# birdnet-team/birdnet-stm32

Measured on AMD Instinct MI355X. Metric: audio chunks/sec (3 s @ 24 kHz), higher is better.
Workload: dtype i8

## Files before the change

### birdnet-stm32_amd/birdnet_stm32/_hip.py

```python

from __future__ import annotations

import ctypes
import os
from ctypes import POINTER, byref, c_char_p, c_float, c_int, c_int32, c_int64, c_size_t, c_void_p

_PKG_ROOT = os.path.dirname(os.path.dirname(os.path.abspath(__file__)))
LIB_PATH = os.path.join(_PKG_ROOT, "lib", "libbirdnet_hip.so")

ABI_VERSION = 2

EXPORTS = (
    "bn_version", "bn_last_error", "bn_device_count", "bn_ctx_create", "bn_ctx_destroy", "bn_model_load",
    "bn_model_free", "bn_model_get_info", "bn_stft_mag", "bn_forward", "bn_infer_audio", "bn_debug_op_output",
    "bn_kernel_names", "bn_profile_enable", "bn_profile_collect", "bn_ingest_resample", "bn_ingest_chunks",
    "bn_pool_scores", "bn_mel_spectrogram", "bn_profile_only", "bn_chunk_peak_normalize", "bn_set_option", "bn_get_option", "bn_ctx_set_option", "bn_ctx_get_option", "bn_ctx_reset_options", "bn_preload_kernels", "bn_host_alloc_pinned", "bn_host_free_pinned", "bn_rank_orders",
    "bn_blob_check", "bn_debug_requant", "bn_stft_mag_exact", "bn_debug_input_bytes", "bn_debug_guard_stats", "bn_debug_tail_form", "bn_debug_mid_form", "bn_debug_mid_plan", "bn_debug_mid_split_giveups",
    "bn_forward_embed", "bn_infer_audio_embed", "bn_model_get_embedding_info", "bn_ingest_resample_span",
    "bn_head_forward", "bn_probe_create", "bn_probe_destroy", "bn_probe_epoch", "bn_probe_loss", "bn_probe_get", "bn_probe_set",
    "bn_probe_sweep_create", "bn_probe_sweep_destroy", "bn_probe_sweep_epoch", "bn_probe_sweep_loss", "bn_probe_sweep_snapshot", "bn_probe_sweep_get",
    "bn_probe_set_loss", "bn_probe_epoch_weighted", "bn_probe_sweep_set_loss", "bn_probe_sweep_epoch_weighted",
    "bn_probe_set_qat", "bn_probe_get_quantized", "bn_probe_scores",
    "bn_short_time_energy", "bn_activity_counts", "bn_search_inv_norms", "bn_search_topk", "bn_augment_inputs",
    "bn_kmeans_assign", "bn_kmeans_accumulate", "bn_kmeans_centroids",
    "bn_tsne_perplexity", "bn_tsne_gradient", "bn_tsne_update",
    "bn_bootstrap_rejections", "bn_bootstrap_counts", "bn_bootstrap_ap", "bn_head_i8_forward", "bn_head_i8_pass_classes",
)

EMB_F32, EMB_I8 = 0, 1
PROBE_ACTIVATIONS = {"sigmoid": 0, "softmax": 1}
PROBE_OPTIMIZERS = {"adam": 0, "adamw": 1, "sgd": 2}
PROBE_LOSSES = {"auto": 0, "focal": 1}
PROBE_QAT_WEIGHTS = {"off": 0, "per_class": 1, "per_tensor": 2}
PROBE_MAX_D, PROBE_MAX_C = 2048, 4096
PROBE_SWEEP_MAX_TRIALS = 64
PROBE_SWEEP_CURRENT, PROBE_SWEEP_SNAPSHOT = 0, 1
HEAD_I8_STEP_ROWS, HEAD_I8_MIN_WG_STEPS, HEAD_I8_MAX_WGS, HEAD_I8_LDS_BYTES = 64, 8, 1024, 160 * 1024



def head_i8_pass_classes(D: int, C: int) -> int:
    v = int(load_library().bn_head_i8_pass_classes(int(D), int(C)))
    check(min(v, 0))
    return v


class ProbeTrialStruct(ctypes.Structure):

    _fields_ = [("optimizer", ctypes.c_int32), ("lr", ctypes.c_float), ("weight_decay", ctypes.c_float), ("clipnorm", ctypes.c_float),
                ("dropout", ctypes.c_float), ("label_smoothing", ctypes.c_float)]


DTYPE_F32, DTYPE_I8 = 0, 1
SEARCH_METRICS = {"cosine": 0, "dot": 1}
SEARCH_MAX_K, SEARCH_MAX_D = 128, 2048
AUGMENT_MAX_MASKS = 4
SEARCH_STEP_ROWS, SEARCH_MIN_WG_STEPS, SEARCH_MAX_WGS = 64, 8, 1024
KMEANS_MAX_K, KMEANS_MAX_D = 4096, 2048
BOOTSTRAP_MAX_N = 32768
KMEANS_LDS_BYTES, KMEANS_MAX_TILE, KMEANS_STEP_ROWS, KMEANS_MIN_WG_STEPS, KMEANS_MAX_WGS, KMEANS_SEGMENT_ROWS = 160 * 1024, 128, 64, 8, 1024, 256
TSNE_TILE_I, TSNE_TILE_J, TSNE_SPLIT_J, TSNE_ROW_LANES, TSNE_MAX_K, TSNE_MAX_N = 256, 1024, 4096, 16, 128, 1 << 21


def kmeans_tile_centroids(D: int, K: int) -> int:
    pitch_bytes = (-(-int(D) // 64) * 64 + 4) * 4
    nt = 1
    while nt < KMEANS_MAX_TILE // 16 and 16 * nt < K:
        nt *= 2
    while nt > 1 and 16 * nt * pitch_bytes > KMEANS_LDS_BYTES:
        nt //= 2
    return 16 * nt


OPTION_NAMES = ("f32_strip", "f32_strip_th", "f32_front_staged", "f32_front2", "f32_pwdw", "f32_tile_slice", "f32_pw_ws", "i8_pwdw", "i8_pw_lds", "i8_pw_forms", "i8_add_tab", "front_tpw", "wave_dwpw", "i8_strip", "i8_strip_mfdw", "i8_strip_th", "i8_dw_pool", "i8_tail_fclds", "i8_tail", "i8_tail_mfdw", "i8_mid",
                "i8_mel_generic", "stft_rowmajor", "stft_exact", "stft_flagcap", "stft_guard", "stft_audit", "stft_minint", "ingest_blk", "ingest_generic")
SCHEDULING_OPTION_NAMES = ("i8_mid_split",)


class BnModelInfo(ctypes.Structure):
    _fields_ = [
        ("dtype", c_int32), ("input_kind", c_int32), ("input_elems", c_int32), ("fft_bins", c_int32),
        ("spec_width", c_int32), ("num_classes", c_int32), ("n_ops", c_int32), ("max_batch", c_int32),
        ("workspace_bytes", c_int64), ("const_bytes", c_int64),
    ]


class HipError(RuntimeError):
    """A libbirdnet_hip call returned a negative status."""


_lib = None


def load_library(path: str | None = None):
    global _lib
    if _lib is not None:
        return _lib
    path = path or os.environ.get("BIRDNET_HIP_LIB", LIB_PATH)
    if not os.path.isfile(path):
        raise RuntimeError(
            f"{path} not found: the HIP extension has not been built. Run `python -c 'import __graft_entry__ as g; "
            "g.build()'` (or `make -C birdnet-stm32_amd/csrc`). There is no CPU fallback for this path."
        )
    import torch

    lib = ctypes.CDLL(path)
    for name in EXPORTS:
        if not hasattr(lib, name):
            raise RuntimeError(f"{path} does not export {name}")
    lib.bn_version.restype = c_int
    lib.bn_last_error.restype = c_char_p
    lib.bn_device_count.restype = c_int
    lib.bn_ctx_create.argtypes = [c_int, c_int, POINTER(c_void_p)]
    lib.bn_ctx_destroy.argtypes = [c_void_p]
    lib.bn_ctx_destroy.restype = None
    lib.bn_model_load.argtypes = [c_void_p, c_char_p, c_size_t, POINTER(c_void_p)]
    lib.bn_model_free.argtypes = [c_void_p]
    lib.bn_model_free.restype = None
    lib.bn_model_get_info.argtypes = [c_void_p, POINTER(BnModelInfo)]
    lib.bn_stft_mag.argtypes = [c_void_p, c_void_p, c_int, c_int, c_int, c_int, c_int, c_int, c_void_p, c_void_p, c_void_p]
    lib.bn_stft_mag_exact.argtypes = lib.bn_stft_mag.argtypes
    lib.bn_debug_input_bytes.argtypes = [c_void_p, c_int, c_void_p, c_void_p]
    lib.bn_debug_guard_stats.argtypes = [c_void_p, c_int, POINTER(c_int64)]
    lib.bn_debug_tail_form.argtypes = [c_void_p, POINTER(c_int), POINTER(c_int)]
    lib.bn_debug_mid_form.argtypes = [c_void_p, POINTER(c_int), POINTER(c_int)]
    lib.bn_debug_mid_plan.argtypes = [c_void_p, POINTER(c_int), c_int]
    lib.bn_debug_mid_split_giveups.argtypes = [c_void_p, POINTER(c_int64)]
    lib.bn_forward.argtypes = [c_void_p, c_void_p, c_void_p, c_int, c_void_p, c_void_p, c_void_p]
    lib.bn_infer_audio.argtypes = [c_void_p, c_void_p, c_int, c_int, c_int, c_void_p, c_void_p, c_void_p]
    lib.bn_forward_embed.argtypes = [c_void_p, c_void_p, c_void_p, c_int, c_void_p, c_void_p, c_void_p, c_int, c_void_p]
    lib.bn_infer_audio_embed.argtypes = [c_void_p, c_void_p, c_int, c_int, c_int, c_void_p, c_void_p, c_void_p, c_int, c_void_p]
    lib.bn_model_get_embedding_info.argtypes = [c_void_p, POINTER(c_int), POINTER(c_int), POINTER(c_float), POINTER(c_int)]
    lib.bn_debug_op_output.argtypes = [c_void_p, c_int, c_int, c_void_p, c_size_t, POINTER(c_size_t), c_void_p]
    lib.bn_kernel_names.restype = c_char_p
    lib.bn_profile_enable.argtypes = [c_void_p, c_int]
    lib.bn_profile_only.argtypes = [c_void_p, c_int]
    lib.bn_chunk_peak_normalize.argtypes = [c_void_p, c_void_p, c_int, c_int, c_float, c_void_p, c_void_p]
    lib.bn_profile_collect.argtypes = [c_void_p, POINTER(ctypes.c_double), POINTER(c_int64), c_int]
    lib.bn_ingest_resample.argtypes = [c_void_p, c_void_p, c_int, c_int, c_void_p, c_void_p, c_int, c_int64, c_int64,
                                       c_void_p, c_int, c_int, c_int, c_int, c_void_p, c_void_p, c_void_p]
    lib.bn_ingest_resample_span.argtypes = [c_void_p, c_void_p, c_int, c_int, c_int64, c_int64, c_int64, c_int64, c_int64, c_void_p,
                                            c_int, c_int, c_int, c_int, c_void_p, c_void_p, c_void_p]
    lib.bn_ingest_chunks.argtypes = [c_void_p, c_void_p, c_void_p, c_void_p, c_void_p, c_void_p, c_int, c_int, c_void_p,
                                     c_void_p]
    lib.bn_pool_scores.argtypes = [c_void_p, c_void_p, c_void_p, c_int, c_int, c_int, c_float, c_void_p, c_void_p]
    lib.bn_mel_spectrogram.argtypes = [c_void_p, c_void_p, c_int, c_int, c_int, c_int, c_int, c_void_p, c_void_p, c_int, c_int, c_int,
                                       ctypes.c_double, c_void_p, c_int, c_void_p, c_void_p, c_void_p]
    lib.bn_blob_check.argtypes = [c_char_p, c_size_t]
    lib.bn_debug_requant.argtypes = [c_void_p, c_void_p, c_void_p, c_void_p, c_int, c_int, c_int, c_void_p, c_void_p]
    lib.bn_set_option.argtypes = [c_char_p, c_int]
    lib.bn_get_option.argtypes = [c_char_p, POINTER(c_int)]
    lib.bn_ctx_set_option.argtypes = [c_void_p, c_char_p, c_int]
    lib.bn_ctx_get_option.argtypes = [c_void_p, c_char_p, POINTER(c_int)]
    lib.bn_ctx_reset_options.argtypes = [c_void_p]
    lib.bn_preload_kernels.argtypes = [c_void_p]
    lib.bn_rank_orders.argtypes = [c_void_p, c_void_p, c_int, c_int, c_void_p, c_void_p, c_void_p]
    lib.bn_short_time_energy.argtypes = [c_void_p, c_void_p, c_void_p, c_void_p, c_void_p, c_void_p, c_int, c_int, c_int, c_void_p, c_void_p]
    lib.bn_activity_counts.argtypes = [c_void_p, c_void_p, c_int, c_int64, c_void_p, c_int, c_float, c_void_p, c_void_p, c_void_p]
    lib.bn_search_inv_norms.argtypes = [c_void_p, c_void_p, c_int, c_int64, c_int, c_int, c_void_p, c_void_p]
    lib.bn_search_topk.argtypes = [c_void_p, c_void_p, c_int, c_int64, c_int, c_int, c_void_p, c_void_p, c_int64, c_void_p, c_int, c_void_p, c_void_p,
                                   c_int, c_void_p, c_void_p, c_void_p]
    lib.bn_kmeans_assign.argtypes = [c_void_p, c_void_p, c_int, c_int64, c_int, c_int, c_void_p, c_void_p, c_void_p, c_int, c_void_p, c_void_p, c_void_p,
                                     c_void_p, c_void_p]
    lib.bn_kmeans_accumulate.argtypes = [c_void_p, c_void_p, c_int, c_int64, c_int, c_int, c_void_p, c_void_p, c_int, c_int, c_void_p, c_void_p, c_void_p]
    lib.bn_kmeans_centroids.argtypes = [c_void_p, c_void_p, c_void_p, c_int, c_int, c_void_p, c_void_p, c_void_p]
    lib.bn_tsne_perplexity.argtypes = [c_void_p, c_void_p, c_int64, c_int, ctypes.c_double, c_void_p, c_void_p, c_void_p]
    lib.bn_tsne_gradient.argtypes = [c_void_p, c_void_p, c_int64, c_void_p, c_void_p, c_void_p, c_float, c_void_p, c_void_p, c_void_p, c_void_p]
    lib.bn_tsne_update.argtypes = [c_void_p, c_void_p, c_void_p, c_void_p, c_void_p, c_int64, c_float, c_float, c_void_p]
    u64 = ctypes.c_uint64
    lib.bn_bootstrap_rejections.argtypes = [c_void_p, u64, u64, u64, u64, ctypes.c_uint32, c_int64, c_int64, c_void_p, c_int64, POINTER(c_int64), c_void_p]
    lib.bn_bootstrap_counts.argtypes = [c_void_p, u64, u64, u64, u64, c_int, c_int, c_void_p, c_void_p, c_void_p]
    lib.bn_bootstrap_ap.argtypes = [c_void_p, u64, u64, u64, u64, c_int, c_int, c_void_p, c_void_p, c_void_p, c_void_p, c_int, c_int, c_void_p, c_void_p, c_void_p]
    lib.bn_augment_inputs.argtypes = [c_void_p, c_void_p, c_int64, c_int, c_int, c_void_p, c_void_p, c_void_p, c_void_p, c_int, c_void_p, c_int, c_int64,
                                      c_void_p, c_void_p]
    lib.bn_host_alloc_pinned.argtypes = [c_void_p, ctypes.c_size_t]
    lib.bn_host_alloc_pinned.restype = c_void_p
    lib.bn_host_free_pinned.argtypes = [c_void_p]
    lib.bn_head_forward.argtypes = [c_void_p, c_void_p, c_int64, c_int, c_void_p, c_void_p, c_int, c_int, c_void_p, c_void_p]
    lib.bn_head_i8_forward.argtypes = [c_void_p, c_void_p, c_int64, c_int, c_void_p, c_void_p, c_void_p, c_void_p, c_int, c_int, c_void_p, c_int, c_float,
                                       c_void_p, c_void_p, c_void_p]
    lib.bn_head_i8_pass_classes.argtypes = [c_int, c_int]
    lib.bn_probe_create.argtypes = [c_void_p, c_int, c_int, c_int, c_int, c_float, c_float, c_float, c_float, ctypes.c_uint32, c_int64,
                                    c_void_p, c_void_p, POINTER(c_void_p), c_void_p]
    lib.bn_probe_destroy.argtypes = [c_void_p]
    lib.bn_probe_destroy.restype = None
    lib.bn_probe_epoch.argtypes = [c_void_p, c_void_p, c_void_p, c_void_p, c_int64, c_int, c_void_p, c_void_p]
    lib.bn_probe_loss.argtypes = [c_void_p, c_void_p, c_void_p, c_int64, c_void_p, c_void_p]
    lib.bn_probe_get.argtypes = [c_void_p, c_void_p, c_void_p, c_void_p]
    lib.bn_probe_set.argtypes = [c_void_p, c_void_p, c_void_p, c_void_p]
    lib.bn_probe_sweep_create.argtypes = [c_void_p, c_int, c_int, c_int, c_int, POINTER(ProbeTrialStruct), ctypes.c_uint32, c_int64, c_void_p, c_void_p,
                                          POINTER(c_void_p), c_void_p]
    lib.bn_probe_sweep_destroy.argtypes = [c_void_p]
    lib.bn_probe_sweep_destroy.restype = None
    lib.bn_probe_sweep_epoch.argtypes = [c_void_p, c_void_p, c_void_p, c_void_p, c_int64, c_int, c_void_p, c_void_p, c_void_p, c_void_p]
    lib.bn_probe_sweep_loss.argtypes = [c_void_p, c_void_p, c_void_p, c_int64, c_void_p, c_void_p, c_void_p]
    lib.bn_probe_sweep_snapshot.argtypes = [c_void_p, c_void_p, c_void_p]
    lib.bn_probe_sweep_get.argtypes = [c_void_p, c_int, c_int, c_void_p, c_void_p, c_void_p]
    lib.bn_probe_set_loss.argtypes = [c_void_p, c_int, c_float]
    lib.bn_probe_epoch_weighted.argtypes = [c_void_p, c_void_p, c_void_p, c_void_p, c_void_p, c_int64, c_int, c_void_p, c_void_p]
    lib.bn_probe_sweep_set_loss.argtypes = [c_void_p, c_int, c_float]
    lib.bn_probe_set_qat.argtypes = [c_void_p, c_int, c_int, c_float, c_int]
    lib.bn_probe_get_quantized.argtypes = [c_void_p, c_void_p, c_void_p]
    lib.bn_probe_scores.argtypes = [c_void_p, c_void_p, c_int64, c_void_p, c_void_p, c_void_p]
    lib.bn_probe_sweep_epoch_weighted.argtypes = [c_void_p, c_void_p, c_void_p, c_void_p, c_void_p, c_int64, c_int, c_void_p, c_void_p, c_void_p, c_void_p]
    if lib.bn_version() != ABI_VERSION:
        raise RuntimeError(f"libbirdnet_hip ABI {lib.bn_version()} != binding ABI {ABI_VERSION}")
    _lib = lib
    return lib

# ... 121 lines not shown
```

### birdnet-stm32_amd/birdnet_stm32/models/runners.py

```python

from __future__ import annotations

import ctypes

import numpy as np

from birdnet_stm32 import _hip
from birdnet_stm32.models import _pack as pk


class HipRunner:

    def __init__(self, plan: pk.Plan, device: int = 0, max_batch: int = 1024, ctx: "_hip.Context | None" = None):
        import torch

        if not torch.cuda.is_available():
            raise RuntimeError("no ROCm device visible: HipRunner has no CPU fallback")
        self._torch = torch
        self.plan = plan
        self.device = torch.device("cuda", device)
        self.ctx = ctx if ctx is not None else _hip.Context(device, max_batch)
        self.model = _hip.Model(self.ctx, plan.to_blob())
        self.lib = self.ctx.lib
        info = self.model.info
# ... 145 lines not shown
    def infer_audio_device(self, audio, hop: int | None = None, return_logits: bool = False, out=None, return_embeddings: bool = False,
                           emb_dtype: str = "float32", emb_out=None):
        torch = self._torch
        self._check_dev(audio, "audio")
        kw = dict(return_embeddings=True, emb_dtype=emb_dtype, emb_out=emb_out) if return_embeddings else {}
        if self.input_kind in (pk.INPUT_MEL, pk.INPUT_WAVEFORM):
            res = self.predict_device(self.model_inputs_device(audio), return_logits=return_logits, **kw)
            if out is not None:
                out.copy_(res[0] if isinstance(res, tuple) else res)
            return res
        B, T = audio.shape
        hop = int(hop) if hop is not None else T // self.spec_width
        scores = out if out is not None else torch.empty((B, self.num_classes), dtype=torch.float32, device=self.device)
        logits = torch.empty_like(scores) if return_logits else None
        emb, code = (None, 0)
        if return_embeddings:
            emb, code = self._emb_buffer(B, emb_dtype, emb_out)
        with torch.cuda.device(self.device):
            for b0 in range(0, B, self.max_batch):
                nb = min(self.max_batch, B - b0)
                if emb is not None:
                    _hip.check(self.lib.bn_infer_audio_embed(self.model.handle, audio[b0:].data_ptr(), nb, T, hop, scores[b0:].data_ptr(),
                                                             logits[b0:].data_ptr() if logits is not None else None, emb[b0:].data_ptr(), code,
                                                             self._stream()))
                    continue
                _hip.check(
                    self.lib.bn_infer_audio(
                        self.model.handle, audio[b0:].data_ptr(), nb, T, hop, scores[b0:].data_ptr(),
                        logits[b0:].data_ptr() if logits is not None else None, self._stream(),
                    )
                )
        if emb is not None:
            return (scores, logits, emb) if return_logits else (scores, emb)
        return (scores, logits) if return_logits else scores

    def stft_device(self, audio, n_fft: int = 512, hop: int | None = None, spec_width: int | None = None, normalize: bool = True,
                    exact: bool = False):
        return stft_device(self.ctx, audio, n_fft, hop, spec_width or self.spec_width, normalize, exact=exact)

    def op_output(self, op_index: int, B: int) -> np.ndarray:
        torch = self._torch
        op = self.plan.ops[op_index]
        per = ctypes.c_size_t()
        _hip.check(self.lib.bn_debug_op_output(self.model.handle, op_index, B, None, 0, ctypes.byref(per), None))
        buf = torch.empty((B, per.value), dtype=torch.uint8, device=self.device)
        _hip.check(self.lib.bn_debug_op_output(self.model.handle, op_index, B, buf.data_ptr(), buf.numel(), ctypes.byref(per), self._stream()))
        torch.cuda.synchronize(self.device)
        raw = buf.cpu().numpy().reshape(-1)
        n = int(np.prod(op.out_shape))
        dt = np.dtype(op.out_dtype)
        return raw[: B * n * dt.itemsize].copy().view(dt).reshape(B, *op.out_shape)

    def input_bytes(self, B: int) -> np.ndarray:
        torch = self._torch
        out = torch.empty((B, self.fft_bins, self.spec_width), dtype=torch.int8, device=self.device)
        _hip.check(self.lib.bn_debug_input_bytes(self.model.handle, B, out.data_ptr(), self._stream()))
        torch.cuda.synchronize(self.device)
        return out.cpu().numpy()

    def guard_stats(self, B: int) -> dict:
        out = (ctypes.c_int64 * 8)()
        _hip.check(self.lib.bn_debug_guard_stats(self.model.handle, B, out))
        return {"listed": int(out[0]), "listed_max": int(out[1]), "dirty_blocks": int(out[2]), "whole_minmax": int(out[3]), "whole_fix": int(out[4]),
                "audited": int(out[5]), "audit_violations": int(out[6]), "interval_min": int(out[7])}

    def tail_form(self) -> tuple[int, int]:
        form, lds = ctypes.c_int(0), ctypes.c_int(0)
        _hip.check(self.lib.bn_debug_tail_form(self.model.handle, ctypes.byref(form), ctypes.byref(lds)))
        return form.value, lds.value

    def mid_form(self) -> tuple[int, int]:
        form, lds = ctypes.c_int(0), ctypes.c_int(0)
        _hip.check(self.lib.bn_debug_mid_form(self.model.handle, ctypes.byref(form), ctypes.byref(lds)))
        return form.value, lds.value

    def mid_plan(self) -> dict | None:
        out = (ctypes.c_int * 64)()
        _hip.check(self.lib.bn_debug_mid_plan(self.model.handle, out, 64))
        if not out[0]:
            return None
        parts = [(out[5 + 6 * i + 2 * k], out[6 + 6 * i + 2 * k]) for i in range(out[4]) for k in range(3) if out[6 + 6 * i + 2 * k]]
        return {"lds_bytes": out[1], "map_bytes": out[2], "bar_off": out[3], "blocks": out[4], "parts": parts}

    def mid_split_giveups(self) -> int:
        n = ctypes.c_int64(0)
        _hip.check(self.lib.bn_debug_mid_split_giveups(self.ctx.handle, ctypes.byref(n)))
        return int(n.value)

    def profile(self, enable: bool) -> None:
        _hip.check(self.lib.bn_profile_enable(self.model.handle, int(bool(enable))))

    def profile_only(self, op_index: int) -> None:
        _hip.check(self.lib.bn_profile_only(self.model.handle, int(op_index)))

    def profile_collect(self) -> list[dict]:
        n = len(self.plan.ops) + 3
        ms = (ctypes.c_double * n)()
        cnt = (ctypes.c_int64 * n)()
        _hip.check(self.lib.bn_profile_collect(self.model.handle, ms, cnt, n))
        rows = []
        for i in range(n):
            if i < len(self.plan.ops):
                op = self.plan.ops[i]
                rows.append({"op": i, "kind": pk.KIND_NAMES[op.kind], "name": op.name, "ms": ms[i], "launches": int(cnt[i]), "p": list(op.p)})
            else:
                kind, name = (("stft512", "stft"), ("stft_minmax_exact", "exact min/max"), ("stft512_f64_list", "float64 pass + redo"))[i - len(self.plan.ops)]
                rows.append({"op": i, "kind": kind, "name": name, "ms": ms[i], "launches": int(cnt[i]), "p": []})
        return rows

    def close(self):
        import sys

        pl = sys.modules.get("birdnet_stm32.audio.pipeline")
        if pl is not None:
            while pl._PREPARE:
                pl._PREPARE.pop().join()
        self.model.close()
        self.ctx.close()


def stft_device(ctx: _hip.Context, audio, n_fft: int = 512, hop: int | None = None, spec_width: int = 256, normalize: bool = True,
                return_minmax: bool = False, exact: bool = False):
    import torch

    if not (audio.is_cuda and audio.dtype == torch.float32 and audio.is_contiguous() and audio.dim() == 2):
        raise ValueError("audio must be a contiguous float32 CUDA tensor [B, T]")
    B, T = audio.shape
    hop = int(hop) if hop is not None else T // spec_width
    spec = torch.empty((B, n_fft // 2 + 1, spec_width), dtype=torch.float32, device=audio.device)
    minmax = torch.empty((B, 2), dtype=torch.float32, device=audio.device)
    with torch.cuda.device(audio.device):
        stream = ctypes.c_void_p(torch.cuda.current_stream(audio.device).cuda_stream)
        fn = ctx.lib.bn_stft_mag_exact if exact else ctx.lib.bn_stft_mag
        _hip.check(fn(ctx.handle, audio.data_ptr(), B, T, n_fft, hop, spec_width, int(normalize), spec.data_ptr(), minmax.data_ptr(), stream))
    return (spec, minmax) if return_minmax else spec


def lower_model_file(model_path: str, keep_all: bool = False, frontend_norm: bool | None = None, fuse: bool = True) -> pk.Plan:
    if model_path.lower().endswith(".tflite"):
        from birdnet_stm32.models._lower_i8 import lower_i8
        from birdnet_stm32.models._tflite_reader import load_tflite

        return lower_i8(load_tflite(model_path), keep_all=keep_all, fuse=fuse)
    from birdnet_stm32.models._keras_loader import load_keras_archive
    from birdnet_stm32.models._lower_f32 import lower_f32

    return lower_f32(load_keras_archive(model_path, frontend_norm=frontend_norm), keep_all=keep_all, fuse=fuse)


def load_model_runner(model_path: str, device: int = 0, max_batch: int = 1024, keep_all: bool = False,
                      frontend_norm: bool | None = None, fuse: bool = True, prepare_pipeline: bool = False) -> HipRunner:
    ctx = None
    if prepare_pipeline:
        import torch

        if not torch.cuda.is_available():
            raise RuntimeError("no ROCm device visible: HipRunner has no CPU fallback")
        from birdnet_stm32.audio.pipeline import prepare_for_evaluate

        ctx = _hip.Context(device, max_batch)
        prepare_for_evaluate(ctx, torch)
    plan = lower_model_file(model_path, keep_all=keep_all, frontend_norm=frontend_norm, fuse=fuse)
    return HipRunner(plan, device=device, max_batch=max_batch, ctx=ctx)
```

### birdnet-stm32_amd/csrc/bn_api.hip

```cpp
#include <hip/hip_runtime.h>

#include <algorithm>
#include <cctype>
#include <cmath>
#include <cstdarg>
#include <cstdio>
#include <cstdlib>
#include <cstring>
#include <string>
#include <vector>

#include "bn_model.h"

namespace {

thread_local std::string g_err;

constexpr int kFft = 512;

struct OptName {
    const char* name;
    int bn::Options::*field;
};
const OptName kOptions[] = {
    {"f32_strip", &bn::Options::f32_strip},       {"f32_strip_th", &bn::Options::f32_strip_th},
    {"f32_front_staged", &bn::Options::f32_front_staged}, {"f32_front2", &bn::Options::f32_front2}, {"f32_pwdw", &bn::Options::f32_pwdw}, {"f32_tile_slice", &bn::Options::f32_tile_slice}, {"f32_pw_ws", &bn::Options::f32_pw_ws}, {"i8_pwdw", &bn::Options::i8_pwdw}, {"i8_pw_lds", &bn::Options::i8_pw_lds}, {"i8_pw_forms", &bn::Options::i8_pw_forms}, {"i8_add_tab", &bn::Options::i8_add_tab}, {"front_tpw", &bn::Options::front_tpw},
    {"wave_dwpw", &bn::Options::wave_dwpw},       {"i8_strip", &bn::Options::i8_strip},
    {"i8_strip_th", &bn::Options::i8_strip_th}, {"i8_dw_pool", &bn::Options::i8_dw_pool}, {"i8_tail_fclds", &bn::Options::i8_tail_fclds},   {"i8_tail", &bn::Options::i8_tail}, {"i8_tail_mfdw", &bn::Options::i8_tail_mfdw}, {"i8_mid", &bn::Options::i8_mid}, {"i8_mid_split", &bn::Options::i8_mid_split},
    {"i8_mel_generic", &bn::Options::i8_mel_generic}, {"stft_rowmajor", &bn::Options::stft_rowmajor},
    {"i8_strip_mfdw", &bn::Options::i8_strip_mfdw}, {"stft_exact", &bn::Options::stft_exact}, {"stft_flagcap", &bn::Options::stft_flagcap}, {"stft_guard", &bn::Options::stft_guard}, {"stft_audit", &bn::Options::stft_audit}, {"stft_minint", &bn::Options::stft_minint},
    {"ingest_blk", &bn::Options::ingest_blk},
    {"ingest_generic", &bn::Options::ingest_generic},
};

bn::Options options_from_env() {
    bn::Options o;
    for (const OptName& e : kOptions) {
        std::string var = "BN_";
        for (const char* c = e.name; *c; ++c) var += (char)toupper((unsigned char)*c);
        if (const char* v = getenv(var.c_str())) o.*(e.field) = atoi(v);
    }
    return o;
}

}

namespace bn {
thread_local Options g_opt;

int fail(int code, const char* fmt, ...) {
    char buf[512];
    va_list ap;
    va_start(ap, fmt);
    vsnprintf(buf, sizeof buf, fmt, ap);
    va_end(ap);
    g_err = buf;
    return code;
}
}
using bn::fail;
using bn::kMaxGridBatch;
using bn::ProfScope;

bn::Options g_opt_default = options_from_env();
std::mutex g_opt_mu;

namespace bn {

int check_device(bn_ctx* ctx) {
    if (!ctx) return fail(BN_ERR_ARG, "null context");
    HIP_TRY(hipSetDevice(ctx->device));
    {
        std::lock_guard<std::mutex> lock(g_opt_mu);
        bn::g_opt = g_opt_default;
        for (const auto& ov : ctx->opt_override) bn::g_opt.*(ov.first) = ov.second;
    }
    return BN_OK;
}

int grow_device_buffer(void** p, size_t* have, size_t need, size_t alloc, hipStream_t s, int code, const char* what) {
    if (need <= *have) return BN_OK;
    HIP_TRY(hipStreamSynchronize(s));
    if (*p) (void)hipFree(*p);
    *p = nullptr;
    *have = 0;
    if (hipMalloc(p, alloc) != hipSuccess) {
        (void)hipGetLastError();
        return fail(code, "hipMalloc of %zu bytes for the %s workspace failed", alloc, what);
    }
    *have = alloc;
    return BN_OK;
}

}
using bn::check_device;
using bn::grow_device_buffer;

namespace {

int row_matrix_check(int dtype, int64_t n, int D, int max_D, int zero_point) {
    if (dtype != BN_DTYPE_F32 && dtype != BN_DTYPE_I8) return fail(BN_ERR_ARG, "unknown dtype %d", dtype);
    if (D < 1 || D > max_D) return fail(BN_ERR_ARG, "embedding width D=%d outside 1..%d", D, max_D);
    if (n < 0 || n > 0x7fffffffLL) return fail(BN_ERR_ARG, "bad row count %lld", (long long)n);
    if (dtype == BN_DTYPE_I8 && (zero_point < -128 || zero_point > 127)) return fail(BN_ERR_ARG, "zero point %d outside -128..127", zero_point);
    return BN_OK;
}

}

extern "C" {

// ... 93 lines not shown
    if (c->d_tsne_work) (void)hipFree(c->d_tsne_work);
    if (c->d_boot_work) (void)hipFree(c->d_boot_work);
    delete c;
}

static int parse_blob(const void* blob, size_t nbytes, BlobHeader& h, std::vector<SlotRec>& slots, std::vector<TensorRec>& tensors,
                      std::vector<OpRec>& ops) {
    if (!blob || nbytes < sizeof(BlobHeader)) return fail(BN_ERR_FORMAT, "blob too small (%zu bytes)", nbytes);
    const char* base = (const char*)blob;
    memcpy(&h, base, sizeof h);
    if (memcmp(h.magic, BN_BLOB_MAGIC, 8) != 0) return fail(BN_ERR_FORMAT, "bad blob magic");
    if (h.version != BN_BLOB_VERSION)
        return fail(BN_ERR_FORMAT, "blob version %u, library expects %u", h.version, BN_BLOB_VERSION);
    auto in_range = [&](uint64_t off, uint64_t len) { return off <= nbytes && len <= nbytes - off; };
    if (!in_range(h.slots_off, (uint64_t)h.n_slots * sizeof(SlotRec)) ||
        !in_range(h.tensors_off, (uint64_t)h.n_tensors * sizeof(TensorRec)) ||
        !in_range(h.ops_off, (uint64_t)h.n_ops * sizeof(OpRec)))
        return fail(BN_ERR_FORMAT, "blob tables exceed the blob size");
    slots.resize(h.n_slots);
    tensors.resize(h.n_tensors);
    ops.resize(h.n_ops);
    if (h.n_slots) memcpy(slots.data(), base + h.slots_off, h.n_slots * sizeof(SlotRec));
    if (h.n_tensors) memcpy(tensors.data(), base + h.tensors_off, h.n_tensors * sizeof(TensorRec));
    if (h.n_ops) memcpy(ops.data(), base + h.ops_off, h.n_ops * sizeof(OpRec));
    for (const TensorRec& t : tensors)
        if (!in_range(t.offset, t.nbytes) || (t.offset & 255)) return fail(BN_ERR_FORMAT, "tensor payload out of range or misaligned");
    for (const SlotRec& sl : slots)
        if (sl.bytes_per_chunk > (1ull << 32)) return fail(BN_ERR_FORMAT, "slot of %llu bytes per chunk", (unsigned long long)sl.bytes_per_chunk);
    for (const OpRec& o : ops) {
        for (int k = 0; k < BN_OP_NT; ++k)
            if (o.t[k] >= (int)h.n_tensors) return fail(BN_ERR_FORMAT, "operator references tensor %d of %u", o.t[k], h.n_tensors);
        const int ids[3] = {o.in0, o.in1, o.out};
        for (int id : ids)
            if (id >= (int)h.n_slots || (id < 0 && id != BN_SLOT_INPUT && id != BN_SLOT_SCORES && id != BN_SLOT_LOGITS && id != BN_SLOT_AUDIO && id != BN_SLOT_NONE))
                return fail(BN_ERR_FORMAT, "operator references slot %d of %u", id, h.n_slots);
    }
    std::string why;
    if (!bn::check_plan(h, slots, tensors, ops, why)) return fail(BN_ERR_FORMAT, "%s", why.c_str());
    return BN_OK;
}

int bn_blob_check(const void* blob, size_t nbytes) {
    BlobHeader h;
    std::vector<SlotRec> slots;
    std::vector<TensorRec> tensors;
    std::vector<OpRec> ops;
    return parse_blob(blob, nbytes, h, slots, tensors, ops);
}

int bn_model_load(bn_ctx* ctx, const void* blob, size_t nbytes, bn_model** out) {
    if (!out) return fail(BN_ERR_ARG, "out is null");
    *out = nullptr;
    if (int rc = check_device(ctx)) return rc;
    bn_model* m = new bn_model();
    m->ctx = ctx;
    if (int rc = parse_blob(blob, nbytes, m->hdr, m->slots, m->tensors, m->ops)) {
        delete m;
        return rc;
    }
    if (int rc = bn::prepare_plan(m, blob)) {
        delete m;
        return rc;
    }
    const BlobHeader& h = m->hdr;
    const char* base = (const char*)blob;
    size_t lo = nbytes, hi = 0;
    for (const TensorRec& t : m->tensors)
        if (t.nbytes) {
            lo = t.offset < lo ? (size_t)t.offset : lo;
            hi = t.offset + t.nbytes > hi ? (size_t)(t.offset + t.nbytes) : hi;
        }
    auto cleanup_fail = [&](int code) {
        bn_model_free(m);
        return code;
    };
    if (hi > lo) {
        m->consts_base = lo;
        m->consts_bytes = hi - lo;
        if (hipMalloc(&m->d_consts, m->consts_bytes) != hipSuccess)
            return cleanup_fail(fail(BN_ERR_NOMEM, "hipMalloc of %zu constant bytes failed", m->consts_bytes));
        if (hipMemcpy(m->d_consts, base + lo, m->consts_bytes, hipMemcpyHostToDevice) != hipSuccess)
            return cleanup_fail(fail(BN_ERR_DEVICE, "copying constants to the device failed"));
    }
    const size_t mb = (size_t)ctx->max_batch;
    m->d_slots.assign(h.n_slots, nullptr);
    for (uint32_t i = 0; i < h.n_slots; ++i) {
        const size_t bytes = mb * m->slots[i].bytes_per_chunk;
        if (bytes == 0) continue;
        if (hipMalloc(&m->d_slots[i], bytes) != hipSuccess)
            return cleanup_fail(fail(BN_ERR_NOMEM, "hipMalloc of %zu workspace bytes (slot %u) failed", bytes, i));
        m->workspace_bytes += bytes;
    }
    if (h.input_kind == BN_INPUT_SPECTROGRAM) {
        const size_t bytes = mb * h.input_elems * sizeof(float);
        if (hipMalloc(&m->d_spec, bytes) != hipSuccess)
            return cleanup_fail(fail(BN_ERR_NOMEM, "hipMalloc of %zu spectrogram workspace bytes failed", bytes));
        m->workspace_bytes += bytes;
    }
    if (m->guard_form_ok && h.dtype == BN_DTYPE_I8) {
        const size_t W = h.spec_width, n_tiles = (W + 15) / 16, t64 = (W + 63) / 64;
        const int cap = 1 << 20;
        size_t off = 0;
        auto take = [&](size_t bytes) {
            const size_t o = off;
            off += (bytes + 255) & ~(size_t)255;
            return o;
        };
        const size_t o_eps = take(mb * W * 4), o_rec = take(mb * n_tiles * bn::kGuardRec * 4), o_list = take(mb * 4), o_cnt = take(mb * 4),
                     o_dirty = take(mb * 4), o_work = take(mb * t64 * 4), o_nw = take(4 * (mb / kMaxGridBatch + 1)), o_hard = take(2 * mb * 4),
                     o_nh = take(8 * (mb / kMaxGridBatch + 1)), o_audit = take(8);
        if (hipMalloc(&m->d_guard, off) != hipSuccess) return cleanup_fail(fail(BN_ERR_NOMEM, "hipMalloc of %zu exactness-pass bytes failed", off));
        m->workspace_bytes += off;
        char* g = m->d_guard;
        m->guard = bn::StftGuard{(float*)(g + o_eps), (int*)(g + o_rec), (float*)(g + o_list), (int*)(g + o_cnt), cap, (int*)(g + o_dirty),
                                 (int*)(g + o_work), (int*)(g + o_nw), (int*)(g + o_hard), (int*)(g + o_nh), (int)mb};
        m->d_audit = (int*)(g + o_audit);
    }
    if (hipMalloc(&m->d_minmax, mb * 2 * sizeof(float)) != hipSuccess ||
        hipMalloc(&m->d_smax, mb * sizeof(float)) != hipSuccess)
        return cleanup_fail(fail(BN_ERR_NOMEM, "hipMalloc of reduction scratch failed"));
    m->workspace_bytes += mb * 3 * sizeof(float);
    if (m->pool8_C) {
        if (hipMalloc(&m->d_pool8, mb * m->pool8_C * sizeof(int32_t)) != hipSuccess)
            return cleanup_fail(fail(BN_ERR_NOMEM, "hipMalloc of pooling scratch failed"));
        if (hipMemset(m->d_pool8, 0, mb * m->pool8_C * sizeof(int32_t)) != hipSuccess) return cleanup_fail(fail(BN_ERR_DEVICE, "clearing the pooling scratch failed"));
        m->workspace_bytes += mb * m->pool8_C * sizeof(int32_t);
    }
    if (m->gap_part_elems) {
        if (hipMalloc(&m->d_gap_part, mb * m->gap_part_elems * sizeof(float)) != hipSuccess)
            return cleanup_fail(fail(BN_ERR_NOMEM, "hipMalloc of pooling scratch failed"));
        m->workspace_bytes += mb * m->gap_part_elems * sizeof(float);
    }
    *out = m;
    return BN_OK;
}

void bn_model_free(bn_model* m) {
    if (!m) return;
    if (m->ctx) (void)hipSetDevice(m->ctx->device);
    (void)hipFree(m->d_consts);
    for (char* p : m->d_slots) (void)hipFree(p);
    (void)hipFree(m->d_spec);
    (void)hipFree(m->d_minmax);
    (void)hipFree(m->d_guard);
    (void)hipFree(m->d_smax);
    (void)hipFree(m->d_gap_part);
    (void)hipFree(m->d_pool8);
    for (auto& r : m->ev_used) {
        (void)hipEventDestroy(r.start);
        (void)hipEventDestroy(r.stop);
    }
    for (hipEvent_t e : m->ev_free) (void)hipEventDestroy(e);
    delete m;
}

int bn_model_get_info(const bn_model* m, bn_model_info* out) {
    if (!m || !out) return fail(BN_ERR_ARG, "null argument");
    out->dtype = (int32_t)m->hdr.dtype;
    out->input_kind = (int32_t)m->hdr.input_kind;
    out->input_elems = (int32_t)m->hdr.input_elems;
    out->fft_bins = (int32_t)m->hdr.fft_bins;
    out->spec_width = (int32_t)m->hdr.spec_width;
    out->num_classes = (int32_t)m->hdr.num_classes;
    out->n_ops = (int32_t)m->hdr.n_ops;
    out->max_batch = m->ctx->max_batch;
    out->workspace_bytes = (int64_t)m->workspace_bytes;
    out->const_bytes = (int64_t)m->consts_bytes;
    return BN_OK;
}

static int stft_mag_impl(bn_ctx* ctx, const float* d_audio, int B, int T, int n_fft, int hop, int W, int normalize, float* d_spec,
                         float* d_minmax, void* stream, bool tile_major, bool exact = false);

int bn_stft_mag(bn_ctx* ctx, const float* d_audio, int B, int T, int n_fft, int hop, int W, int normalize,
                float* d_spec, float* d_minmax, void* stream) {
    return stft_mag_impl(ctx, d_audio, B, T, n_fft, hop, W, normalize, d_spec, d_minmax, stream, false);
}

int bn_stft_mag_exact(bn_ctx* ctx, const float* d_audio, int B, int T, int n_fft, int hop, int W, int normalize,
                      float* d_spec, float* d_minmax, void* stream) {
    return stft_mag_impl(ctx, d_audio, B, T, n_fft, hop, W, normalize, d_spec, d_minmax, stream, false, true);
}

static int stft_mag_impl(bn_ctx* ctx, const float* d_audio, int B, int T, int n_fft, int hop, int W, int normalize, float* d_spec,
                         float* d_minmax, void* stream, bool tile_major, bool exact) {
    if (int rc = check_device(ctx)) return rc;
    if (!d_audio || !d_spec || !d_minmax) return fail(BN_ERR_ARG, "null device pointer");
    if (n_fft != kFft) return fail(BN_ERR_UNSUPPORTED, "n_fft=%d: only 512 is implemented", n_fft);
    if (B < 0 || T <= 0 || W <= 0 || hop <= 0) return fail(BN_ERR_ARG, "bad shape B=%d T=%d hop=%d W=%d", B, T, hop, W);
    if (1 + T / hop < W)
        return fail(BN_ERR_ARG, "T=%d hop=%d gives %d frames, fewer than spec_width=%d", T, hop, 1 + T / hop, W);
    if (B == 0) return BN_OK;
    hipStream_t s = (hipStream_t)stream;
    const size_t per_chunk = (size_t)(kFft / 2 + 1) * W;
    for (int b0 = 0; b0 < B; b0 += kMaxGridBatch) {
        const int nb = B - b0 < kMaxGridBatch ? B - b0 : kMaxGridBatch;
        bn::launch_minmax_init(d_minmax + 2 * (size_t)b0, nb, s);
        if (exact)
            bn::launch_stft512_f64(ctx->tables, d_audio + (size_t)b0 * T, nb, T, hop, W, d_spec + b0 * per_chunk, d_minmax + 2 * (size_t)b0, s,
                                   tile_major);
        else
            bn::launch_stft512(ctx->tables, d_audio + (size_t)b0 * T, nb, T, hop, W, d_spec + b0 * per_chunk,
                               d_minmax + 2 * (size_t)b0, s, tile_major);
        if (normalize)
            bn::launch_spec_normalize(d_spec + b0 * per_chunk, d_minmax + 2 * (size_t)b0, nb, (int)per_chunk, s);
    }
    HIP_TRY(hipGetLastError());
    return BN_OK;
}

int bn_mel_spectrogram(bn_ctx* ctx, const float* d_audio, int B, int T, int n_fft, int hop, int W, const float* d_mel_w,
                       const int32_t* d_mel_bands, int n_mels, int mode, int mag_scale, double pcen_b, const float* d_dct,
                       int n_mfcc, float* d_work, float* d_out, void* stream) {
    if (int rc = check_device(ctx)) return rc;
    if (!d_audio || !d_mel_w || !d_mel_bands || !d_work || !d_out) return fail(BN_ERR_ARG, "null device pointer");
    if (n_fft != kFft) return fail(BN_ERR_UNSUPPORTED, "n_fft=%d: only 512 is implemented", n_fft);
    if (B < 0 || T <= 0 || W <= 0 || hop <= 0 || n_mels <= 0) return fail(BN_ERR_ARG, "bad shape B=%d T=%d hop=%d W=%d mels=%d", B, T, hop, W, n_mels);
    if (1 + T / hop < W)
        return fail(BN_ERR_ARG, "T=%d hop=%d gives %d frames, fewer than spec_width=%d", T, hop, 1 + T / hop, W);
    if (mode < BN_SPEC_MEL || mode > BN_SPEC_MFCC) return fail(BN_ERR_ARG, "unknown spectrogram mode %d", mode);
    if (mag_scale < BN_MAG_NONE || mag_scale > BN_MAG_DB) return fail(BN_ERR_ARG, "unknown mag_scale %d", mag_scale);
    if (mode != BN_SPEC_MEL) mag_scale = BN_MAG_NONE;
    if (mode == BN_SPEC_MFCC && (!d_dct || n_mfcc <= 0 || n_mfcc > n_mels)) return fail(BN_ERR_ARG, "mfcc needs 0 < n_mfcc <= n_mels and a DCT matrix");
// ... 116 lines not shown
                                 d_emb ? (char*)d_emb + b0 * D * esize : nullptr, emb_dtype, (hipStream_t)stream, d_audio + (size_t)b0 * T, T, hop};
            if (int rc = bn::run_plan(m, ra)) return rc;
        }
        return BN_OK;
    }
    if (int rc = check_device(m->ctx)) return rc;
    if (!d_audio || !d_scores) return fail(BN_ERR_ARG, "null device pointer");
    if (B == 0) return BN_OK;
    const bool tiled = m->spec_tiled_ok && !bn::g_opt.stft_rowmajor;
    hipStream_t s = (hipStream_t)stream;
    const size_t in_stride = m->hdr.input_elems, C = m->hdr.num_classes;
    const bool i8 = m->hdr.dtype == BN_DTYPE_I8;
    const int exact_opt = i8 ? bn::g_opt.stft_exact : 0;
    const bool guarded = exact_opt == 2 && tiled && m->d_guard && !bn::g_opt.i8_mel_generic && W % 16 == 0 && W <= 1024;
    int rc = BN_OK;
    if (guarded) {
        if (T <= 0 || hop <= 0 || 1 + T / hop < W) rc = fail(BN_ERR_ARG, "T=%d hop=%d gives %d frames, fewer than spec_width=%d", T, hop, hop > 0 ? 1 + T / hop : 0, W);
        if (m->d_audit) HIP_TRY(hipMemsetAsync(m->d_audit, 0, 2 * sizeof(int), s));
        for (int b0 = 0; rc == BN_OK && b0 < B; b0 += kMaxGridBatch) {
            const int nb = B - b0 < kMaxGridBatch ? B - b0 : kMaxGridBatch;
            bn::StftGuard g = bn::guard_slice(m, (size_t)b0, bn::SpecStage{tiled, true, d_audio + (size_t)b0 * T, T, hop});
            {
                ProfScope prof(m, (int)m->ops.size(), s);
                bn::launch_stft512(m->ctx->tables, d_audio + (size_t)b0 * T, nb, T, hop, W, m->d_spec + b0 * in_stride, m->d_minmax + 2 * (size_t)b0, s,
                                   true, &g);
            }
            ProfScope prof(m, (int)m->ops.size() + 1, s);
            bn::launch_stft_minmax_exact(m->ctx->tables, d_audio + (size_t)b0 * T, nb, T, hop, W, m->d_spec + b0 * in_stride, true, g,
                                         m->d_minmax + 2 * (size_t)b0, s);
        }
    } else {
        ProfScope prof(m, (int)m->ops.size(), s);
        rc = stft_mag_impl(m->ctx, d_audio, B, T, kFft, hop, W, 0, m->d_spec, m->d_minmax, stream, tiled, exact_opt != 0);
    }
    if (rc == BN_OK) {
        for (int b0 = 0; b0 < B; b0 += kMaxGridBatch) {
            const int nb = B - b0 < kMaxGridBatch ? B - b0 : kMaxGridBatch;
            bn::RunArgs ra{m->d_spec + b0 * in_stride, m->d_minmax + 2 * (size_t)b0, nb, d_scores + b0 * C, d_logits ? d_logits + b0 * C : nullptr,
                           d_emb ? (char*)d_emb + b0 * D * esize : nullptr, emb_dtype, s};
            ra.slot_b0 = (size_t)b0;
            ra.spec = bn::SpecStage{tiled, guarded, d_audio + (size_t)b0 * T, T, hop};
            rc = bn::run_plan(m, ra);
            if (rc != BN_OK) break;
        }
    }
    m->last_tiled = tiled;
    m->last_B = rc == BN_OK ? B : 0;
    return rc;
}

extern "C" {

int bn_debug_tail_form(const bn_model* m, int* form, int* lds_bytes) {
    if (!m || !form || !lds_bytes) return fail(BN_ERR_ARG, "null argument");
    *form = 0;
    *lds_bytes = 0;
    for (size_t oi = 0; oi < m->ops.size(); ++oi) {
        if (m->ops[oi].kind != BN_OP_I8_TAIL || !m->prep[oi]->ok) continue;
        const bn::OpPrep& pr = *m->prep[oi];
        *form = pr.alt_ok ? 2 : 1;
        *lds_bytes = pr.alt_ok ? pr.chain.lds_bytes : pr.tail.lds_bytes;
    }
    return BN_OK;
}

int bn_debug_mid_form(const bn_model* m, int* form, int* lds_bytes) {
    if (!m || !form || !lds_bytes) return fail(BN_ERR_ARG, "null argument");
    *form = 0;
    *lds_bytes = 0;
    for (size_t oi = 0; oi < m->ops.size(); ++oi)
        if (m->ops[oi].kind == BN_OP_I8_MID && m->prep[oi]->ok) {
            *form = 1;
            *lds_bytes = m->prep[oi]->chain.lds_bytes;
        }
    return BN_OK;
}

int bn_debug_mid_plan(const bn_model* m, int* out, int n) {
    if (!m || !out || n < 1) return fail(BN_ERR_ARG, "null argument");
    out[0] = 0;
    for (size_t oi = 0; oi < m->ops.size(); ++oi)
        if (m->ops[oi].kind == BN_OP_I8_MID && m->prep[oi]->ok && m->prep[oi]->alt_ok) {
            if (!bn::tail2_plan_dump(m->prep[oi]->resident, out, n)) return fail(BN_ERR_ARG, "n=%d is too small for the plan", n);
            break;
        }
    return BN_OK;
}

int bn_debug_mid_split_giveups(bn_ctx* ctx, int64_t* count) {
    if (!ctx || !count) return fail(BN_ERR_ARG, "null argument");
    if (int rc = check_device(ctx)) return rc;
    const long n = bn::tail2_giveups();
    if (n < 0) return fail(BN_ERR_DEVICE, "could not read the chunk barriers' give-up counter");
    *count = n;
    return BN_OK;
}

int bn_debug_guard_stats(bn_model* m, int B, int64_t* out) {
    if (!m || !out) return fail(BN_ERR_ARG, "null argument");
    if (int rc = check_device(m->ctx)) return rc;
    if (!m->d_guard) return fail(BN_ERR_UNSUPPORTED, "the plan has no exactness pass");
    if (B <= 0 || B > m->last_B || B > kMaxGridBatch) return fail(BN_ERR_ARG, "B=%d: the last bn_infer_audio call left %d spectrograms", B, m->last_B);
    HIP_TRY(hipDeviceSynchronize());
    std::vector<int> cnt((size_t)B);
    int nw = 0, nh[2] = {0, 0};
    HIP_TRY(hipMemcpy(cnt.data(), m->guard.count, (size_t)B * sizeof(int), hipMemcpyDeviceToHost));
    HIP_TRY(hipMemcpy(&nw, m->guard.n_work, sizeof(int), hipMemcpyDeviceToHost));
    HIP_TRY(hipMemcpy(nh, m->guard.n_hard, 2 * sizeof(int), hipMemcpyDeviceToHost));
    int64_t total = 0, mx = 0;
    for (int c : cnt) {
        c %= m->guard.cap + 1;
        total += c;
        if (c > mx) mx = c;
    }
    out[0] = total;
    out[1] = mx;
    out[2] = nw;
    out[3] = nh[0];
    out[4] = nh[1];
    int au[2] = {0, 0};
    if (m->d_audit) HIP_TRY(hipMemcpy(au, m->d_audit, sizeof au, hipMemcpyDeviceToHost));
    out[5] = au[0];
    out[6] = au[1];
    std::vector<float> lo((size_t)B);
    HIP_TRY(hipMemcpy(lo.data(), m->guard.mn_lo, (size_t)B * sizeof(float), hipMemcpyDeviceToHost));
    int64_t wide = 0;
    for (float v : lo) wide += v >= 0.0f;
    out[7] = wide;
    return BN_OK;
}

int bn_debug_input_bytes(bn_model* m, int B, int8_t* d_out, void* stream) {
    if (!m || !d_out) return fail(BN_ERR_ARG, "null argument");
    if (int rc = check_device(m->ctx)) return rc;
    namespace k = bn::op::i8_dwpw;
    const OpRec* first = nullptr;
    for (const OpRec& o : m->ops)
        if (o.in0 == BN_SLOT_INPUT && o.kind == BN_OP_I8_DWPW && o.p[k::q_at_load] && o.p[k::transposed]) first = &o;
    if (!first || !m->d_spec) return fail(BN_ERR_UNSUPPORTED, "the plan's first operator is not the mel mixer with QUANTIZE fused into its load");
    if (B <= 0 || B > m->last_B || B > kMaxGridBatch) return fail(BN_ERR_ARG, "B=%d: the last bn_infer_audio call left %d spectrograms", B, m->last_B);
    bn::launch_spec_bytes(m->d_spec, m->d_minmax, B, (int)m->hdr.spec_width, m->last_tiled, first->f[k::qscale], first->p[k::qzp], d_out, (hipStream_t)stream);
    HIP_TRY(hipGetLastError());
    return BN_OK;
}

int bn_ingest_resample(bn_ctx* ctx, const void* d_pcm, int sample_format, int channels, const int64_t* d_in_off,
                       const int64_t* d_out_off, int n_windows, int64_t max_in_len, int64_t max_out_len, const float* d_taps,
                       int up, int down, int taps_per_phase, int n_pre_remove, float* d_mono, float* d_peak, void* stream) {
    if (int rc = check_device(ctx)) return rc;
    if (!d_pcm || !d_in_off || !d_out_off || !d_mono || !d_peak) return fail(BN_ERR_ARG, "null device pointer");
    if (sample_format < BN_PCM_S16 || sample_format > BN_PCM_F32) return fail(BN_ERR_ARG, "unknown sample format %d", sample_format);
    if (channels < 1 || channels > 8)
        return fail(BN_ERR_UNSUPPORTED, "%d channels: the channel mean is implemented for 1..8 channels", channels);
    if (n_windows < 0 || max_in_len < 0 || max_out_len < 0 || up < 1 || down < 1 || taps_per_phase < 0 || n_pre_remove < 0)
        return fail(BN_ERR_ARG, "bad ingest geometry");
    if (taps_per_phase > 0 && !d_taps) return fail(BN_ERR_ARG, "null filter");
    if (taps_per_phase == 0 && up != down) return fail(BN_ERR_ARG, "up=%d down=%d needs a filter", up, down);
    if (n_windows == 0 || max_out_len == 0) return BN_OK;
    if (n_windows > 65535) return fail(BN_ERR_ARG, "at most 65535 windows per call");
    if ((double)(max_out_len + n_pre_remove + 4096) * down >= 4294967296.0 || (double)max_in_len * up >= 4294967296.0)
        return fail(BN_ERR_UNSUPPORTED, "window too long for the 32-bit polyphase index (%lld samples, up=%d, down=%d)",
                    (long long)max_in_len, up, down);
    const size_t lds = bn::ingest_resample_lds_bytes(up, down, taps_per_phase, bn::ingest_resample_block(up, down, taps_per_phase));
    const bool fast_kernel = (up == 1 && (down == 2 || down == 4)) || (up > 1 && up <= 256 && (taps_per_phase == 21 || taps_per_phase == 29 || taps_per_phase == 39));
    if (lds > (fast_kernel ? 64 : 156) * 1024)
        return fail(BN_ERR_UNSUPPORTED, "resampling ratio %d/%d needs %zu bytes of LDS per workgroup (limit %d)", up, down, lds, (fast_kernel ? 64 : 156) * 1024);
// ... 605 lines not shown
```

### birdnet-stm32_amd/csrc/bn_chain_plan.cpp

```cpp
#include "bn_chain_plan.h"

#include <algorithm>
#include <vector>

namespace bn {
namespace {

constexpr int kLdsCap = 160 * 1024;
#ifdef BN_TAIL_STAMPS
constexpr int kStampBytes = 16;
#else
constexpr int kStampBytes = 0;
#endif

struct Span {
    int b, e;
};
bool overlap(Span p, Span q) { return p.b < q.e && q.b < p.e; }
int first_fit(std::vector<Span>& used, int bytes, int cap) {
    bytes = (bytes + 15) & ~15;
    int pos = 0;
    for (;;) {
        bool moved = false;
        for (const Span& s : used)
// ... 89 lines not shown
    return true;
}

long tail_const_words(const Tail8Args& a) {
    long need = 0;
    auto upto = [&](long off, long words) { need = off + words > need ? off + words : need; };
    for (int i = 0; i < a.n_layers; ++i) {
        const Tail8Layer& L = a.L[i];
        upto(L.g_w, (long)L.Cin * L.Cout / 4);
        upto(L.g_dwc, (long)L.Cin * 7);
        upto(L.g_pwc, (long)L.Cout * 4);
        if (L.has_add) upto(L.g_lut, 512);
    }
    upto(a.g_fcw, (long)a.NC * a.C / 4);
    upto(a.g_fcb, a.NC);
    upto(a.g_fcm, a.NC);
    upto(a.g_fcs, a.NC);
    if (a.g_hlut >= 0) upto(a.g_hlut, 64);
    return need;
}

namespace {

Span dw_span(const Tail2Layer& L, bool first) { return {L.dw_off, L.dw_off + tail2_dw_bytes(L, first)}; }
int tail2_map_bytes(const Tail2Layer& L, bool first, int G) {
    return std::max(first ? 0 : G * L.H * L.W * (L.Cin + 16), G * L.OH * L.OW * (L.Cout + 16));
}
void tail2_place_counters(Tail2Args& a) {
    a.bar_off = (a.lds_bytes + 15) & ~15;
    if (a.bar_off + 16 > kLdsCap) a.bar_off = -1;
    else a.lds_bytes = a.bar_off + 16;
}

}

bool tail2_plan(const int32_t* desc, int n_words, int n_layers, Tail2Args& a, bool mid) {
    constexpr int LW = kTail2LayerWords, CAP = kLdsCap - kStampBytes;
    const int HW = mid ? 0 : kTailHeadWords, G = mid ? kMidG : kTailG;
    if (n_layers < 1 || n_layers > 8 || n_words != LW * n_layers + HW) return false;
    a.n_layers = n_layers;
    int lds_need = 0;
    Span prev_pw{0, 0}, map_last{0, 0};
    auto grow = [&](int end) { lds_need = end > lds_need ? end : lds_need; };
    for (int attempt = 0; attempt < 2; ++attempt) {
        lds_need = 0;
        prev_pw = {0, 0};
        for (int i = 0; i < n_layers; ++i) {
            const int32_t* d = desc + LW * i;
            Tail2Layer& L = a.L[i];
            read_layer(d, L);
            L.res_m = d[20]; L.res_c_lo = d[21]; L.res_c_hi = d[22]; L.res_k = d[23]; L.g_cst = d[24];
            const bool first = i == 0;
            if (!(mid ? shape_ok(a.L, i, kMidShapes) : shape_ok(a.L, i, kTailShapes))) return false;
            if (L.g_cst < 0 || (L.g_cst & 3)) return false;
            if (first && L.zp_in != -128) return false;
            if (!int8_range(L.dw_lo, L.dw_hi) || L.pw_lo > L.pw_hi) return false;
            if (!L.has_add && !int8_range(L.pw_lo, L.pw_hi)) return false;
            if (L.has_add && (!int8_range(L.add_lo, L.add_hi) || L.add_e < 1 || L.add_e > 22 || L.add_m < 0 || L.res_m < 0 || L.res_k < 3 || L.res_k > 19))
                return false;
            if (tail2_dw_bytes(L, first) / 16 > kTail2MaxDw16) return false;
            const Span map{0, tail2_map_bytes(L, first, G)};
            L.x_off = first ? -1 : 0;
            L.y_off = 0;
            std::vector<Span> used{map};
            if (prev_pw.e > prev_pw.b) used.push_back(prev_pw);
            L.zp_off = first ? 0 : first_fit(used, L.Cin + 16, CAP);
            if (L.zp_off < 0) return false;
            L.dw_off = first && attempt ? (CAP - tail2_dw_bytes(L, first)) & ~15 : first_fit(used, tail2_dw_bytes(L, first), CAP);
            if (L.dw_off < 0) return false;
            used = {map, dw_span(L, first)};
            if (!first) used.push_back({L.zp_off, L.zp_off + L.Cin + 16});
            L.pw_off = first_fit(used, tail2_pw_bytes(L), CAP);
            if (L.pw_off < 0) return false;
            prev_pw = {L.pw_off, L.pw_off + tail2_pw_bytes(L)};
            grow(map.e); grow(dw_span(L, first).e); grow(prev_pw.e);
        }
        const Tail2Layer& last = a.L[n_layers - 1];
        map_last = {0, G * last.OH * last.OW * (last.Cout + 16)};
        if (!overlap(dw_span(a.L[0], true), map_last) && !overlap(dw_span(a.L[0], true), prev_pw)) break;
        if (attempt) return false;
    }
    const Tail2Layer& last = a.L[n_layers - 1];
    a.resident = 0;
    a.bar_off = -1;
    a.fcw_off = -1;
    if (mid) {
        a.P = last.OH * last.OW;
        a.C = last.Cout;
        a.lds_bytes = lds_need;
        tail2_place_counters(a);
        return a.C % 16 == 0;
    }
    read_head(desc + LW * n_layers, a);
    if (a.g_fcw < 0 || a.g_fcb < 0 || a.g_hlut < -1 || (a.g_fcw & 3) || (a.g_fcb & 3)) return false;
    if (!int8_range(a.fc_lo, a.fc_hi)) return false;
    if (a.P != last.OH * last.OW || a.C != last.Cout || a.C % 64 || a.C > 256 || a.NC < 1 || (a.NC + 15) / 16 > kTail2Waves) return false;
    std::vector<Span> used{map_last, dw_span(a.L[0], true)};
    a.mean_off = first_fit(used, kTailG * last.Cout, CAP);
    if (a.mean_off < 0) return false;
    grow(a.mean_off + kTailG * last.Cout);
    a.lds_bytes = lds_need;
    tail2_place_counters(a);
    return true;
}

bool tail2_plan_resident(Tail2Args& a) {
    if (a.n_layers < 1 || a.n_layers > 8) return false;
    int map_bytes = 0;
    for (int i = 0; i < a.n_layers; ++i) map_bytes = std::max(map_bytes, tail2_map_bytes(a.L[i], i == 0, kMidG));
    std::vector<Span> used{{0, map_bytes}};
    for (int i = 0; i < a.n_layers; ++i) {
        Tail2Layer& L = a.L[i];
        if (tail2_dw_bytes(L, i == 0) / 16 > kTail2MaxDw16 || tail2_pw_bytes(L) / 16 > kTail2MaxDw16) return false;
        if ((L.dw_off = first_fit(used, tail2_dw_bytes(L, i == 0), kLdsCap)) < 0) return false;
        if ((L.pw_off = first_fit(used, tail2_pw_bytes(L), kLdsCap)) < 0) return false;
        L.zp_off = 0;
        if (i > 0 && (L.zp_off = first_fit(used, L.Cin + 16, kLdsCap)) < 0) return false;
    }
    if ((a.bar_off = first_fit(used, 16, kLdsCap)) < 0) return false;
    for (size_t i = 0; i < used.size(); ++i)
        for (size_t j = i + 1; j < used.size(); ++j)
            if (overlap(used[i], used[j])) return false;
    const Tail2Layer& last = a.L[a.n_layers - 1];
    if (last.OH != 16 || last.OW != 32 || last.Cout != 64 || a.P != 16 * 32 || a.C != 64) return false;
    int end = 0;
    for (const Span& u : used) end = std::max(end, u.e);
    a.lds_bytes = end;
    a.resident = 1;
    return end <= kLdsCap;
}

bool tail2_plan_dump(const Tail2Args& a, int* out, int n) {
    if (n < 5 + 6 * a.n_layers) return false;
    int map_bytes = 0;
    for (int i = 0; i < a.n_layers; ++i) {
        const Tail2Layer& L = a.L[i];
        map_bytes = std::max(map_bytes, tail2_map_bytes(L, i == 0, kMidG));
        int* o = out + 5 + 6 * i;
        o[0] = L.dw_off; o[1] = tail2_dw_bytes(L, i == 0); o[2] = L.pw_off; o[3] = tail2_pw_bytes(L); o[4] = L.zp_off; o[5] = i == 0 ? 0 : L.Cin + 16;
    }
    out[0] = a.resident; out[1] = a.lds_bytes; out[2] = map_bytes; out[3] = a.bar_off; out[4] = a.n_layers;
    return true;
}

long tail2_const_words(const Tail2Args& a, bool mid) {
    long need = 0;
    auto upto = [&](long off, long words) { need = off + words > need ? off + words : need; };
    for (int i = 0; i < a.n_layers; ++i) upto(a.L[i].g_cst, (tail2_dw_bytes(a.L[i], i == 0) + tail2_pw_bytes(a.L[i])) / 4);
    if (mid) return need;
    const long nct = (a.NC + 15) / 16;
    upto(a.g_fcw, nct * (a.C / 64) * 256);
    upto(a.g_fcb, nct * 48);
    if (a.g_hlut >= 0) upto(a.g_hlut, 64);
    return need;
}

}
```

### birdnet-stm32_amd/csrc/bn_chain_plan.h

```cpp
#pragma once
#include <stdint.h>

#if defined(__HIPCC__)
#define BN_HOST_DEVICE __host__ __device__
#else
#define BN_HOST_DEVICE
#endif

namespace bn {

constexpr int kTailG = 4;
constexpr int kTailWaves = 16;
constexpr int kTailThreads = 64 * kTailWaves;
constexpr int kTailLayerWords = 24;
constexpr int kTailHeadWords = 16;
struct Tail8Layer {
    int H, W, Cin, Cout, S, OH, OW, pt, pl, has_add;
    int zp_in, dw_lo, dw_hi, pw_lo, pw_hi;
    int add_m, add_c1, add_e, add_lo, add_hi;
    int g_w, g_dwc, g_pwc, g_lut;
    int x_off, y_off, w_off, dwc_off, pwc_off, lut_off, zp_off;
};
struct Tail8Args {
    const int8_t* x;
    float* scores;
    float* logits;
    const int32_t* cst;
    int B, n_layers, NC, P, C;
    int mean_zp_in, mean_mult, mean_shift, mean_zp_out, mean_off;
    int fc_zp_out, fc_lo, fc_hi, g_fcw, g_fcb, g_fcm, g_fcs, g_hlut, head_zp_fc, head_zp_out;
    float s_fc, s_head;
    int lds_bytes;
    int fcw_off;
    Tail8Layer L[8];};
bool tail_plan(const int32_t* desc, int n_words, int n_layers, Tail8Args& a);
long tail_const_words(const Tail8Args& a);

constexpr int kTail2Waves = 8;
constexpr int kTail2Threads = 64 * kTail2Waves;
constexpr int kTail2LayerWords = 32;
struct Tail2Layer {
    int H, W, Cin, Cout, S, OH, OW, pt, pl, has_add;
    int zp_in, dw_lo, dw_hi, pw_lo, pw_hi;
    int add_m, add_c1, add_e, add_lo, add_hi;
    int res_m, res_c_lo, res_c_hi, res_k;
    int g_cst;
    int x_off, y_off, dw_off, pw_off, zp_off;
};
constexpr int kMidG = 2;
struct Tail2Args {
    const int8_t* x;
    int8_t* y;
    float* scores;
    float* logits;
    const int32_t* cst;
    int B, n_layers, NC, P, C;
    int mean_zp_in, mean_mult, mean_shift, mean_zp_out, mean_off;
    int fc_zp_out, fc_lo, fc_hi, g_fcw, g_fcb, g_fcm, g_fcs, g_hlut, head_zp_fc, head_zp_out;
    float s_fc, s_head;
    int lds_bytes;
    int fcw_off;
    int bar_off;
    int resident;
    Tail2Layer L[8];};
constexpr int kTail2MaxDw16 = 7 * kTail2Threads;
BN_HOST_DEVICE inline int tail2_dw_bytes(const Tail2Layer& L, bool first) { return (L.Cin / 16) * (3 * 1024 + (first ? 8 : 5) * 64); }
BN_HOST_DEVICE inline int tail2_pw_bytes(const Tail2Layer& L) { return (L.Cin + 63) / 64 * 64 * L.Cout + (L.Cout / 16) * 5 * 64; }
bool tail2_plan(const int32_t* desc, int n_words, int n_layers, Tail2Args& a, bool mid = false);
bool tail2_plan_resident(Tail2Args& a);
bool tail2_plan_dump(const Tail2Args& a, int* out, int n);
long tail2_const_words(const Tail2Args& a, bool mid = false);

}
```

### birdnet-stm32_amd/csrc/bn_i8_tail2.hip

```cpp
#include "bn_tail_common.h"

namespace bn {
namespace {

#ifdef BN_TAIL_STAMPS
__device__ long long* g_tail2_stamps = nullptr;
__device__ long long* g_mid2_stamps = nullptr;
#define BN_T2STAMP(i) do { if ((i) != 7) st[i] = (long long)__builtin_amdgcn_s_memrealtime(); } while (0)
#else
#define BN_T2STAMP(i) do {} while (0)
#endif

__device__ __forceinline__ long upair(uint32_t lo, uint32_t hi) { return (long)(((unsigned long)hi << 32) | lo); }

template <int MAXP>
__device__ __forceinline__ void part_request(const int32_t* src, unsigned char* dst, int n16, int tid) {
    const int wave = __builtin_amdgcn_readfirstlane(tid >> 6);
#pragma unroll
    for (int i = 0; i < MAXP; ++i) {
        const int idx = i * kTail2Threads + tid;
        if (idx < n16)
            __builtin_amdgcn_global_load_lds((const __attribute__((address_space(1))) void*)(src + 4 * (size_t)idx),
                                             (__attribute__((address_space(3))) void*)(dst + (i * kTail2Threads + wave * 64) * 16), 16, 0, 0);
    }
}
__device__ unsigned g_tail2_giveups = 0;
#ifdef BN_TAIL_STAMPS
constexpr bool kStamped = true;
#else
constexpr bool kStamped = false;
#endif
template <int WPC>
__device__ __forceinline__ void chunk_barrier(unsigned char* lds, int bar_off, int slot, unsigned& seq) {
    unsigned* ctr = reinterpret_cast<unsigned*>(lds + bar_off) + slot;
    seq += 1;
    const unsigned target = (unsigned)WPC * seq;
    asm volatile("s_waitcnt lgkmcnt(0)" ::: "memory");
    __builtin_amdgcn_fence(__ATOMIC_RELEASE, "workgroup", "local");
    if ((threadIdx.x & 63) == 0) __hip_atomic_fetch_add(ctr, 1u, __ATOMIC_RELAXED, __HIP_MEMORY_SCOPE_WORKGROUP);
    bool done = false;
#pragma unroll 1
    for (int spins = 0; spins < (1 << 20); ++spins) {
        const unsigned v = (unsigned)__builtin_amdgcn_readfirstlane((int)__hip_atomic_load(ctr, __ATOMIC_RELAXED, __HIP_MEMORY_SCOPE_WORKGROUP));
        if ((int)(v - target) >= 0) {
            done = true;
            break;
        }
        __builtin_amdgcn_s_sleep(1);
    }
    if (!done && (threadIdx.x & 63) == 0) atomicAdd(&g_tail2_giveups, 1u);
    __builtin_amdgcn_fence(__ATOMIC_ACQUIRE, "workgroup", "local");
}

__device__ __forceinline__ int rq_signed(int x, int m2, long c, int e_packed, int e) {
    const int hi = (int)(((long)x * (long)m2 + c) >> 32);
    const int s = hi + x + (x >> 31);
    return ashr_byte(e_packed, s, e);
}

template <bool EMB>
__device__ __forceinline__ void tail2_head(const Tail2Args& a_, unsigned char* lds, int chunk0, int stamp_slot = -1) {
#ifdef BN_TAIL_STAMPS
    long long st[8] = {0, 0, 0, 0, 0, 0, 0, 0};
    st[0] = (long long)__builtin_amdgcn_s_memrealtime();
#endif
    const Tail2Args* ap = (const Tail2Args*)__builtin_amdgcn_kernarg_segment_ptr();
    asm volatile("" : "+s"(ap));
    const Tail2Args& a = *ap;
    (void)a_;
    int tid = threadIdx.x;
    asm volatile("" : "+v"(tid));
    const int lane = tid & 63, wave = __builtin_amdgcn_readfirstlane(tid >> 6);
    const int n = lane & 15, g = lane >> 4;
    const Tail2Layer& L = a.L[a.n_layers - 1];
    const int C = a.C, KS = C / 64, nct = (a.NC + 15) / 16, pitch = C + 16;
    const bool fc_wave = wave < nct;
    const v4i* gw = reinterpret_cast<const v4i*>(a.cst + a.g_fcw) + (fc_wave ? wave : nct - 1) * KS * 64 + lane;
    const v4i af0 = gw[0], af1 = KS > 1 ? gw[64] : af0, af2 = KS > 2 ? gw[128] : af0, af3 = KS > 3 ? gw[192] : af0;
    const v4i* fc = reinterpret_cast<const v4i*>(a.cst + a.g_fcb) + (fc_wave ? wave : nct - 1) * 12 + g;
    const v4i fc_b = fc[0], fc_mu = fc[4], fc_sh = fc[8];
    for (int i = tid; i < kTailG * (C / 4); i += kTail2Threads) {
        const int gq = i / (C / 4), cq = i - gq * (C / 4);
        const int* src = reinterpret_cast<const int*>(lds + L.y_off + gq * a.P * pitch + 4 * cq);
        int s0 = 0, s1 = 0, s2 = 0, s3 = 0;
        int k = 0;
        for (; k + 8 <= a.P; k += 8) {
            int x[8];
#pragma unroll
            for (int u = 0; u < 8; ++u) x[u] = src[(k + u) * (pitch / 4)];
#pragma unroll
            for (int u = 0; u < 8; ++u) { s0 += (int)(int8_t)x[u]; s1 += (int)(int8_t)(x[u] >> 8); s2 += (int)(int8_t)(x[u] >> 16); s3 += x[u] >> 24; }
        }
        for (; k < a.P; ++k) {
            const int x = src[k * (pitch / 4)];
            s0 += (int)(int8_t)x; s1 += (int)(int8_t)(x >> 8); s2 += (int)(int8_t)(x >> 16); s3 += x >> 24;
        }
        const int q[4] = {mean_q(s0, a.P, a.mean_zp_in, a.mean_mult, a.mean_shift, a.mean_zp_out), mean_q(s1, a.P, a.mean_zp_in, a.mean_mult, a.mean_shift, a.mean_zp_out),
                          mean_q(s2, a.P, a.mean_zp_in, a.mean_mult, a.mean_shift, a.mean_zp_out), mean_q(s3, a.P, a.mean_zp_in, a.mean_mult, a.mean_shift, a.mean_zp_out)};
        reinterpret_cast<int*>(lds + a.mean_off)[i] = pack4(q);
        if constexpr (EMB) {
            const EmbOut& eo = reinterpret_cast<const WithEmb<Tail2Args>*>(ap)->e;
            const int chunk = chunk0 + gq;
            if (chunk < a.B) {
                const size_t e = (size_t)chunk * C + 4 * cq;
                if (eo.f32)
                    *reinterpret_cast<float4*>(reinterpret_cast<float*>(eo.emb) + e) =
                        make_float4((float)(q[0] - eo.zp) * eo.scale, (float)(q[1] - eo.zp) * eo.scale, (float)(q[2] - eo.zp) * eo.scale,
                                    (float)(q[3] - eo.zp) * eo.scale);
                else
                    *reinterpret_cast<int*>(reinterpret_cast<int8_t*>(eo.emb) + e) = pack4(q);
            }
        }
    }
    __syncthreads();
#ifdef BN_TAIL_STAMPS
    st[4] = (long long)__builtin_amdgcn_s_memrealtime();
#endif
    if (fc_wave) {
        v4i acc = fc_b;
        const v4i mu = fc_mu, sh = fc_sh;
        const unsigned char* mv = lds + a.mean_off + (n & (kTailG - 1)) * C + 16 * g;
        acc = __builtin_amdgcn_mfma_i32_16x16x64_i8(af0, *reinterpret_cast<const v4i*>(mv), acc, 0, 0, 0);
        if (KS > 1) acc = __builtin_amdgcn_mfma_i32_16x16x64_i8(af1, *reinterpret_cast<const v4i*>(mv + 64), acc, 0, 0, 0);
        if (KS > 2) acc = __builtin_amdgcn_mfma_i32_16x16x64_i8(af2, *reinterpret_cast<const v4i*>(mv + 128), acc, 0, 0, 0);
        if (KS > 3) acc = __builtin_amdgcn_mfma_i32_16x16x64_i8(af3, *reinterpret_cast<const v4i*>(mv + 192), acc, 0, 0, 0);
        const int chunk = chunk0 + n;
        if (n < kTailG && chunk < a.B) {
#pragma unroll
            for (int r = 0; r < 4; ++r) {
                const int j = 16 * wave + 4 * g + r;
                if (j < a.NC) {
                    const int qv = clampi(mbqm(acc[r], mu[r], sh[r]) + a.fc_zp_out, a.fc_lo, a.fc_hi);
                    const size_t o = (size_t)chunk * a.NC + j;
                    if (a.logits) a.logits[o] = (float)(qv - a.head_zp_fc) * a.s_fc;
                    if (a.g_hlut >= 0) {
                        const int ov = reinterpret_cast<const int8_t*>(a.cst + a.g_hlut)[qv + 128];
                        a.scores[o] = (float)(ov - a.head_zp_out) * a.s_head;
                    } else {
                        a.scores[o] = (float)(qv - a.head_zp_fc) * a.s_fc;
                    }
                }
            }
        }
    }
#ifdef BN_TAIL_STAMPS
    if (stamp_slot >= 0 && g_tail2_stamps && (threadIdx.x & 63) == 0) {
        long long* o = g_tail2_stamps + ((size_t)stamp_slot * kTail2Waves + (threadIdx.x >> 6)) * 8;
        o[0] = st[0]; o[4] = st[4];
    }
#endif
}

template <int G, int CIN, int COUT, int S, int H, int W, bool ADD, bool SRCG, bool RES = false>
__device__ __forceinline__ void tail2_block(const Tail2Layer& L, const Tail2Args& a, unsigned char* lds, int chunk0, int nxi, unsigned& seq, int stamp_slot = -1) {
#ifdef BN_TAIL_STAMPS
    long long st[8] = {0, 0, 0, 0, 0, 0, 0, 0};
#endif
    BN_T2STAMP(0);
    constexpr int KS = (CIN + 63) / 64, NCT = CIN / 16, NT = COUT / 16;
    constexpr int PIN = CIN + 16, POUT = COUT + 16;
    constexpr int OH = H / S, OW = W / S, PER_CHUNK = OH * OW;
    constexpr int TILES = G * PER_CHUNK / 16;
    static_assert(TILES % kTail2Waves == 0, "tiles per wave");
    constexpr int TPW = TILES / kTail2Waves;
    constexpr int UPW = TPW < 4 ? TPW : 4;
    constexpr int PASSES = TPW / UPW;
    static_assert(TPW % UPW == 0, "passes");
    constexpr int TR = OW == 8 ? 2 : 1;
    constexpr int STRIPS = OW == 8 ? 1 : OW / 16;
    constexpr int WPC = kTail2Waves / G;
    static_assert(kTail2Waves % G == 0 && WPC % STRIPS == 0 && (WPC / STRIPS) * TPW * TR == OH, "a wave's tiles: one strip of one chunk");
    constexpr int PSTEP = TR * OW;
    constexpr int NR = (UPW - 1) * TR * S + 3;
    constexpr int PT = S == 1 ? 1 : 0, PL = PT;
    constexpr int DWK = SRCG ? 8 : 5;
    constexpr int W_BYTES = KS * 64 * COUT, DWA_BYTES = NCT * 3 * 1024, DWC_BYTES = NCT * DWK * 64, PWC_BYTES = NT * 5 * 64;
    constexpr int PW16 = (W_BYTES + PWC_BYTES) / 16, PWP = (PW16 + kTail2Threads - 1) / kTail2Threads;
    int tid = threadIdx.x;
    asm volatile("" : "+v"(tid));
    const int lane = tid & 63;
    const int wave = __builtin_amdgcn_readfirstlane(tid >> 6);
    const int n = lane & 15, g = lane >> 4;

    if constexpr (!RES) part_request<PWP>(a.cst + L.g_cst + (DWA_BYTES + DWC_BYTES) / 4, lds + L.pw_off, PW16, tid);

    const v4i* wl = reinterpret_cast<const v4i*>(lds + L.pw_off) + lane;
    const v4i* dwa = reinterpret_cast<const v4i*>(lds + L.dw_off) + lane;
    const v4i* dwc = reinterpret_cast<const v4i*>(lds + L.dw_off + DWA_BYTES) + g;
    const v4i* pwc = reinterpret_cast<const v4i*>(lds + L.pw_off + W_BYTES) + g;
    const int dw_lo = L.dw_lo, dw_hi = L.dw_hi, pw_lo = L.pw_lo, pw_hi = L.pw_hi;

    const int gch = wave / WPC, wi = wave % WPC;
    const int cx0 = (wi % STRIPS) * 16;
    const int oy_base = (wi / STRIPS) * TPW * TR;
    const int lr = OW == 8 ? n >> 3 : 0, ox = OW == 8 ? n & 7 : cx0 + n;
    int chunk = chunk0 + gch;
    if (chunk >= a.B) chunk = a.B - 1;
    const __amdgpu_buffer_rsrc_t rs = __builtin_amdgcn_make_buffer_rsrc(
        const_cast<int8_t*>(a.x) + (SRCG ? (size_t)chunk * H * W * CIN : 0), 0, SRCG ? H * W * CIN : 0, 0x00020000);
    v4i bf[TPW][KS];
    if constexpr (CIN % 64 != 0) {
#pragma unroll
        for (int t = 0; t < TPW; ++t) bf[t][KS - 1] = (v4i){0, 0, 0, 0};
    }
#pragma unroll
    for (int pass = 0; pass < PASSES; ++pass) {
    const int oy0 = oy_base + pass * UPW * TR;
    int raddr[NR];
#pragma unroll
    for (int r = 0; r < NR; ++r) {
        const int iy = (oy0 + lr) * S - PT + r, ix = ox * S - PL + g;
        const bool ok = g < 3 && (unsigned)iy < (unsigned)H && (unsigned)ix < (unsigned)W;
        if constexpr (SRCG) raddr[r] = ok ? (iy * W + ix) * CIN : 0x40000000;
        else raddr[r] = ok ? L.x_off + ((gch * H + iy) * W + ix) * PIN : L.zp_off;
    }
    int bkind[UPW];
#pragma unroll
    for (int t = 0; t < UPW; ++t) {
        const bool right = ox == OW - 1, bottom = oy0 + t * TR + lr == OH - 1;
        bkind[t] = SRCG ? (right ? (bottom ? 7 : 5) : (bottom ? 6 : 0)) * 4 : 0;
    }

    constexpr int AHEAD = NCT < 4 ? NCT : 4;
    v4i grow[SRCG ? NCT : 1][SRCG ? NR : 1];
    if constexpr (SRCG) {
#pragma unroll
        for (int ct = 0; ct < AHEAD && ct < NCT; ++ct)
#pragma unroll
            for (int r = 0; r < NR; ++r) grow[ct][r] = __builtin_bit_cast(v4i, __builtin_amdgcn_raw_buffer_load_b128(rs, raddr[r] + 16 * ct, 0, 0));
    }
    constexpr int NB0 = SRCG ? UPW : 1;
    v4i af[2][3], brow[2][NR], acc[2][UPW], b0[2][NB0], rqm[2], rq01[2], rq23[2];
    int rqe[2];
    auto request = [&](int ct) {
        const int b = ct & 1;
#pragma unroll
        for (int dy = 0; dy < 3; ++dy) af[b][dy] = dwa[(ct * 3 + dy) * 64];
#pragma unroll
        for (int r = 0; r < NR; ++r) {
            if constexpr (SRCG) {
                brow[b][r] = grow[ct][r];
                if (ct + AHEAD < NCT) grow[ct + AHEAD][r] = __builtin_bit_cast(v4i, __builtin_amdgcn_raw_buffer_load_b128(rs, raddr[r] + 16 * (ct + AHEAD), 0, 0));
            } else {
                brow[b][r] = *reinterpret_cast<const v4i*>(lds + raddr[r] + 16 * ct);
            }
        }
        const v4i* dc = dwc + ct * DWK * 4;
#pragma unroll
        for (int t = 0; t < NB0; ++t) b0[b][t] = SRCG ? dc[bkind[t]] : dc[0];
    };
    auto request_rq = [&](int ct) {
        const int b = ct & 1;
        const v4i* dc = dwc + ct * DWK * 4;
        rqm[b] = dc[4]; rq01[b] = dc[8]; rq23[b] = dc[12];
        rqe[b] = reinterpret_cast<const int*>(dc + 16)[0];
    };
    request(0);
#pragma unroll
    for (int ct = 0; ct <= NCT; ++ct) {
        if (ct + 1 < NCT) request(ct + 1);
        if (ct < NCT) {
            const int b = ct & 1;
            request_rq(ct);
#pragma unroll
            for (int dy = 0; dy < 3; ++dy)
#pragma unroll
                for (int t = 0; t < UPW; ++t)
                    acc[b][t] = __builtin_amdgcn_mfma_i32_16x16x64_i8(af[b][dy], brow[b][t * TR * S + dy], dy ? acc[b][t] : b0[b][SRCG ? t : 0], 0, 0, 0);
        }
        if (ct > 0) {
            const int pt = ct - 1, b = pt & 1, c = b;
            const long cc[4] = {pair(rq01[c].x, rq01[c].y), pair(rq01[c].z, rq01[c].w), pair(rq23[c].x, rq23[c].y), pair(rq23[c].z, rq23[c].w)};
#pragma unroll
            for (int t = 0; t < UPW; ++t) {
                int qv[4];
#pragma unroll
                for (int e = 0; e < 4; ++e) qv[e] = med3(rq_hi(acc[b][t][e], rqm[c][e], cc[e], rqe[c], e), dw_lo, dw_hi);
                bf[pass * UPW + t][pt >> 2][pt & 3] = pack4(qv);
            }
        }
        __builtin_amdgcn_sched_barrier(0);
    }
    }
    BN_T2STAMP(1);
    if constexpr (RES) {
        if constexpr (!SRCG) chunk_barrier<WPC>(lds, a.bar_off, gch, seq);
    } else {
#ifdef BN_TAIL_STAMPS
        if (a.bar_off >= 0) chunk_barrier<WPC>(lds, a.bar_off, gch, seq);
        BN_T2STAMP(3);
#endif
        __syncthreads();
    }
    BN_T2STAMP(4);
    const Tail2Layer& N = a.L[nxi < 0 ? 0 : nxi];
    if constexpr (!RES) {
        const int nx_n16 = nxi < 0 ? 0 : tail2_dw_bytes(N, nxi == 0) / 16;
        part_request<kTail2MaxDw16 / kTail2Threads>(a.cst + N.g_cst, lds + N.dw_off, nx_n16, tid);
    }

    const int add_m = L.add_m, add_e1 = L.add_e - 1;
    const long add_c = rq64(L.add_c1);
    const uint32_t res_m = (uint32_t)L.res_m;
    const long res_c = upair((uint32_t)L.res_c_lo, (uint32_t)L.res_c_hi);
    const int res_k = L.res_k;
#pragma unroll
    for (int pass = 0; pass < PASSES; ++pass) {
    const int pbase = (gch * OH + oy_base + pass * UPW * TR) * OW + (OW == 8 ? 0 : cx0) + n;
    v4i paf[2][KS], pb0[2], pacc[2][UPW], pm[2], pc01[2], pc23[2];
    int pe1[2], pres[2][ADD ? UPW : 1];
    auto request_a = [&](int nt) {
        const int b = nt & 1;
#pragma unroll
        for (int ks = 0; ks < KS; ++ks) paf[b][ks] = wl[(nt * KS + ks) * 64];
        pb0[b] = pwc[nt * 20];
    };
    auto request_e = [&](int nt) {
        const int b = nt & 1;
        const v4i* pc = pwc + nt * 20;
        pm[b] = pc[4]; pc01[b] = pc[8]; pc23[b] = pc[12];
        pe1[b] = reinterpret_cast<const int*>(pc + 16)[0];
        if constexpr (ADD) {
#pragma unroll
            for (int t = 0; t < UPW; ++t) pres[b][t] = *reinterpret_cast<const int*>(lds + L.x_off + (pbase + PSTEP * t) * PIN + 4 * g + 16 * nt);
        }
    };
    auto matrix = [&](int nt) {
        const int b = nt & 1;
#pragma unroll
        for (int ks = 0; ks < KS; ++ks)
#pragma unroll
            for (int t = 0; t < UPW; ++t) pacc[b][t] = __builtin_amdgcn_mfma_i32_16x16x64_i8(paf[b][ks], bf[pass * UPW + t][ks], ks ? pacc[b][t] : pb0[b], 0, 0, 0);
    };
    request_a(0);
    request_e(0);
    if (NT > 1) request_a(1);
    matrix(0);
#pragma unroll
    for (int nt = 0; nt < NT; ++nt) {
        const int b = nt & 1;
        if (nt + 1 < NT) {
            request_e(nt + 1);
            matrix(nt + 1);
        }
        if (nt + 2 < NT) request_a(nt + 2);
        const long cc[4] = {pair(pc01[b].x, pc01[b].y), pair(pc01[b].z, pc01[b].w), pair(pc23[b].x, pc23[b].y), pair(pc23[b].z, pc23[b].w)};
#pragma unroll
        for (int t = 0; t < UPW; ++t) {
            const int p = pbase + PSTEP * t;
            const int xr = ADD ? pres[b][t] ^ (int)0x80808080u : 0;
            int qv[4];
#pragma unroll
            for (int e = 0; e < 4; ++e) {
                if constexpr (ADD) {
                    const int v = rq_signed(pacc[b][t][e], pm[b][e], cc[e], pe1[b], e);
                    const uint32_t xt = (uint32_t)perm(0, xr, ((uint32_t)e << 24) | 0x000c0c0cu);
                    const int f = (int)((uint32_t)(((unsigned long)xt * (unsigned long)res_m + (unsigned long)res_c) >> 32) >> res_k);
                    const int total = (v << 19) + f;
                    qv[e] = med3((int)(((long)total * (long)add_m + add_c) >> 32) >> add_e1, L.add_lo, L.add_hi);
                } else {
                    qv[e] = med3(rq_hi(pacc[b][t][e], pm[b][e], cc[e], pe1[b], e), pw_lo, pw_hi);
                }
            }
            *reinterpret_cast<int*>(lds + L.y_off + p * POUT + 4 * g + 16 * nt) = pack4(qv);
        }
        __builtin_amdgcn_sched_barrier(0);
    }
    }
    BN_T2STAMP(2);
    if constexpr (RES) {
        (void)N;
        if (nxi > 0) chunk_barrier<WPC>(lds, a.bar_off, gch, seq);
    } else {
        if (nxi > 0 && tid < (N.Cin + 16) / 4) reinterpret_cast<int*>(lds + N.zp_off)[tid] = (N.zp_in & 0xff) * 0x01010101;
#ifdef BN_TAIL_STAMPS
        if (a.bar_off >= 0) chunk_barrier<WPC>(lds, a.bar_off, gch, seq);
        BN_T2STAMP(5);
#endif
        __syncthreads();
    }
    BN_T2STAMP(6);
#ifdef BN_TAIL_STAMPS
    long long* const sbuf = G == kMidG ? g_mid2_stamps : g_tail2_stamps;
    if (stamp_slot >= 0 && sbuf && (threadIdx.x & 63) == 0) {
        long long* o = sbuf + ((size_t)stamp_slot * kTail2Waves + (threadIdx.x >> 6)) * 8;
        for (int i = 0; i < 7; ++i) o[i] = st[i];
    }
#endif
}

template <bool EMB>
__device__ __forceinline__ void tail2_main(const Tail2Args& a) {
    extern __shared__ __attribute__((aligned(16))) unsigned char lds[];
    const int ngroups = (a.B + kTailG - 1) / kTailG;
    unsigned seq = 0;
#ifdef BN_TAIL_STAMPS
    if (threadIdx.x < 4 && a.bar_off >= 0) reinterpret_cast<unsigned*>(lds + a.bar_off)[threadIdx.x] = 0;
#endif
    {
        part_request<kTail2MaxDw16 / kTail2Threads>(a.cst + a.L[0].g_cst, lds + a.L[0].dw_off, tail2_dw_bytes(a.L[0], true) / 16, (int)threadIdx.x);
        __syncthreads();
    }
    for (int grp = blockIdx.x; grp < ngroups; grp += gridDim.x) {
        const int chunk0 = grp * kTailG;
        const bool more = grp + (int)gridDim.x < ngroups;
        for (int li = 0; li < a.n_layers; ++li) {
            const Tail2Layer& L = a.L[li];
            const bool last = li == a.n_layers - 1;
            const Tail2Layer& N = a.L[last ? 0 : li + 1];
            const int nx = last ? (more ? 0 : -1) : li + 1;
            (void)N;
            int slot = -1;
#ifdef BN_TAIL_STAMPS
            const int gi = (grp - (int)blockIdx.x) / (int)gridDim.x;
            if ((int)blockIdx.x < 8 && gi < 4 && li < 8 && g_tail2_stamps) slot = ((int)blockIdx.x * 4 + gi) * 8 + li;
#endif
            if (L.Cin == 64) tail2_block<kTailG, 64, 128, 2, 16, 32, false, true>(L, a, lds, chunk0, nx, seq, slot);
            else if (L.Cin == 128 && L.Cout == 128) tail2_block<kTailG, 128, 128, 1, 8, 16, true, false>(L, a, lds, chunk0, nx, seq, slot);
            else if (L.Cin == 128) tail2_block<kTailG, 128, 256, 2, 8, 16, false, false>(L, a, lds, chunk0, nx, seq, slot);
            else tail2_block<kTailG, 256, 256, 1, 4, 8, true, false>(L, a, lds, chunk0, nx, seq, slot);
        }
        int hslot = -1;
#ifdef BN_TAIL_STAMPS
        const int gi = (grp - (int)blockIdx.x) / (int)gridDim.x;
        if ((int)blockIdx.x < 8 && gi < 4 && g_tail2_stamps) hslot = ((int)blockIdx.x * 4 + gi) * 8 + 6;
#endif
        tail2_head<EMB>(a, lds, chunk0, hslot);
        __syncthreads();
#ifdef BN_TAIL_STAMPS
        if (hslot >= 0 && (threadIdx.x & 63) == 0) g_tail2_stamps[((size_t)hslot * kTail2Waves + (threadIdx.x >> 6)) * 8 + 6] = (long long)__builtin_amdgcn_s_memrealtime();
#endif
    }
}

__global__ __launch_bounds__(kTail2Threads) void i8_tail2_kernel(Tail2Args a) { tail2_main<false>(a); }
__global__ __launch_bounds__(kTail2Threads) void i8_tail2_emb_kernel(WithEmb<Tail2Args> w) { tail2_main<true>(w.a); }

template <bool RES>
__device__ __forceinline__ void mid2_main(const Tail2Args& a) {
    extern __shared__ __attribute__((aligned(16))) unsigned char lds[];
    const int ngroups = (a.B + kMidG - 1) / kMidG;
    unsigned seq = 0;
    if (RES || kStamped) {
        if (threadIdx.x < 4 && a.bar_off >= 0) reinterpret_cast<unsigned*>(lds + a.bar_off)[threadIdx.x] = 0;
    }
    if constexpr (RES) {
        for (int li = 0; li < a.n_layers; ++li) {
            const Tail2Layer& L = a.L[li];
            const int dw16 = tail2_dw_bytes(L, li == 0) / 16;
            part_request<kTail2MaxDw16 / kTail2Threads>(a.cst + L.g_cst, lds + L.dw_off, dw16, (int)threadIdx.x);
            part_request<kTail2MaxDw16 / kTail2Threads>(a.cst + L.g_cst + 4 * dw16, lds + L.pw_off, tail2_pw_bytes(L) / 16, (int)threadIdx.x);
            if (li > 0 && (int)threadIdx.x < (L.Cin + 16) / 4) reinterpret_cast<int*>(lds + L.zp_off)[threadIdx.x] = (L.zp_in & 0xff) * 0x01010101;
        }
    } else {
        part_request<kTail2MaxDw16 / kTail2Threads>(a.cst + a.L[0].g_cst, lds + a.L[0].dw_off, tail2_dw_bytes(a.L[0], true) / 16, (int)threadIdx.x);
    }
    __syncthreads();
    for (int grp = blockIdx.x; grp < ngroups; grp += gridDim.x) {
        const int chunk0 = grp * kMidG;
        const bool more = grp + (int)gridDim.x < ngroups;
        for (int li = 0; li < a.n_layers; ++li) {
            const Tail2Layer& L = a.L[li];
            const bool last = li == a.n_layers - 1;
            const int nx = last ? (more ? 0 : -1) : li + 1;
            int slot = -1;
#ifdef BN_TAIL_STAMPS
            const int gi = (grp - (int)blockIdx.x) / (int)gridDim.x;
            if ((int)blockIdx.x < 8 && gi < 4 && li < 8 && g_mid2_stamps) slot = ((int)blockIdx.x * 4 + gi) * 8 + li;
#endif
            if (li == 0) tail2_block<kMidG, 32, 64, 2, 32, 64, false, true, RES>(L, a, lds, chunk0, nx, seq, slot);
            else tail2_block<kMidG, 64, 64, 1, 16, 32, true, false, RES>(L, a, lds, chunk0, nx, seq, slot);
        }
        const Tail2Layer& L = a.L[a.n_layers - 1];
        const int c16 = L.Cout / 16, per = a.P * c16;
        if constexpr (RES) {
            constexpr int WPC = kTail2Waves / kMidG, OW = 32, C = 64;
            const int lane = (int)threadIdx.x & 63, wave = __builtin_amdgcn_readfirstlane((int)threadIdx.x >> 6);
            const int gq = wave / WPC, wi = wave % WPC, cx0 = (wi % 2) * 16, oy0 = (wi / 2) * 8;
            if (chunk0 + gq < a.B) {
#pragma unroll
                for (int r = 0; r < 8; ++r) {
                    const int pos = (oy0 + r) * OW + cx0 + (lane >> 2);
                    reinterpret_cast<v4i*>(a.y + ((size_t)(chunk0 + gq) * (16 * OW) + pos) * C)[lane & 3] =
                        *reinterpret_cast<const v4i*>(lds + L.y_off + (gq * (16 * OW) + pos) * (C + 16) + 16 * (lane & 3));
                }
            }
        } else {
            for (int i = threadIdx.x; i < kMidG * per; i += kTail2Threads) {
                const int gq = i / per, r = i - gq * per, pos = r / c16, c = r - pos * c16;
                if (chunk0 + gq < a.B)
                    reinterpret_cast<v4i*>(a.y + ((size_t)(chunk0 + gq) * a.P + pos) * L.Cout)[c] =
                        *reinterpret_cast<const v4i*>(lds + L.y_off + (gq * a.P + pos) * (L.Cout + 16) + 16 * c);
            }
            __syncthreads();
        }
    }
}

__global__ __launch_bounds__(kTail2Threads) void i8_mid2_kernel(Tail2Args a) {
    if (a.resident) mid2_main<true>(a);
    else mid2_main<false>(a);
}

}

#ifdef BN_TAIL_STAMPS
extern "C" __attribute__((visibility("default"))) int bn_debug_tail2_stamps(long long* d_buf) {
    return hipMemcpyToSymbol(HIP_SYMBOL(g_tail2_stamps), &d_buf, sizeof d_buf) == hipSuccess ? 0 : -1;
}
extern "C" __attribute__((visibility("default"))) int bn_debug_mid2_stamps(long long* d_buf) {
    return hipMemcpyToSymbol(HIP_SYMBOL(g_mid2_stamps), &d_buf, sizeof d_buf) == hipSuccess ? 0 : -1;
}
#endif

long tail2_giveups() {
    unsigned n = 0;
    if (hipDeviceSynchronize() != hipSuccess || hipMemcpyFromSymbol(&n, HIP_SYMBOL(g_tail2_giveups), sizeof n) != hipSuccess) return -1;
    return (long)n;
}

bool launch_i8_tail2(Tail2Args a, hipStream_t s, const EmbOut* emb) {
    const void* k = emb ? reinterpret_cast<const void*>(i8_tail2_emb_kernel) : reinterpret_cast<const void*>(i8_tail2_kernel);
    if (!ensure_dynamic_lds(k, 160 * 1024)) return false;
    const int ngroups = (a.B + kTailG - 1) / kTailG;
    const int grid = ngroups < 256 ? ngroups : 256;
    if (emb)
        hipLaunchKernelGGL(i8_tail2_emb_kernel, dim3(grid), dim3(kTail2Threads), (size_t)a.lds_bytes, s, WithEmb<Tail2Args>{a, *emb});
    else
        hipLaunchKernelGGL(i8_tail2_kernel, dim3(grid), dim3(kTail2Threads), (size_t)a.lds_bytes, s, a);
    return true;
}

bool launch_i8_mid2(Tail2Args a, hipStream_t s) {
    if (!ensure_dynamic_lds(reinterpret_cast<const void*>(i8_mid2_kernel), 160 * 1024)) return false;
    const int ngroups = (a.B + kMidG - 1) / kMidG;
    const int grid = ngroups < 256 ? ngroups : 256;
    hipLaunchKernelGGL(i8_mid2_kernel, dim3(grid), dim3(kTail2Threads), (size_t)a.lds_bytes, s, a);
    return true;
}


void preload_i8_tail2() {
    hipFuncAttributes at;
    (void)hipFuncGetAttributes(&at, reinterpret_cast<const void*>(&i8_tail2_kernel));
}

}
```

### birdnet-stm32_amd/csrc/bn_kernels.h

```cpp
#pragma once
#include <hip/hip_runtime.h>
#include <stdint.h>

#include <map>
#include <mutex>
#include <string>
#include <utility>
#include <vector>

#include "bn_blob.h"
#include "bn_chain_plan.h"

namespace bn {

struct Options {
    int f32_strip = 1;
    int f32_strip_th = 0;
    int f32_front_staged = 1;
    int i8_pwdw = 0;
    int f32_pw_ws = 1;
    int f32_tile_slice = 0;
    int f32_pwdw = 2;
    int f32_front2 = 1;
    int front_tpw = 0;
    int wave_dwpw = 1;
    int i8_strip = 1;
    int i8_strip_th = 0;
    int i8_dw_pool = 1;
    int i8_pw_lds = 1;
    int i8_pw_forms = 1;
    int i8_add_tab = 1;
    int i8_tail_fclds = 1;
    int i8_tail = 1;
    int i8_mid = 1;
    int i8_tail_mfdw = 1;
    int i8_mel_generic = 0;
    int stft_rowmajor = 0;
    int i8_mid_split = 1;
    int i8_strip_mfdw = 1;
    int stft_exact = 2;
    int stft_guard = 0;
    int stft_audit = 0;
    int stft_minint = 1;
    int stft_flagcap = 1022;
    int ingest_blk = 0;
    int ingest_generic = 0;
};
extern thread_local Options g_opt;

inline bool ensure_dynamic_lds(const void* kernel, size_t bytes) {
    static std::mutex mu;
    static std::map<std::pair<const void*, int>, size_t> allowed;
    int dev = 0;
    if (hipGetDevice(&dev) != hipSuccess) return false;
    std::lock_guard<std::mutex> lock(mu);
    size_t& have = allowed[{kernel, dev}];
    if (bytes <= have) return true;
    if (hipFuncSetAttribute(kernel, hipFuncAttributeMaxDynamicSharedMemorySize, (int)bytes) != hipSuccess) {
        (void)hipGetLastError();
        return false;
    }
    have = bytes;
    return true;
}

bool check_plan(const BlobHeader& h, const std::vector<SlotRec>& slots, const std::vector<TensorRec>& tensors,
                const std::vector<OpRec>& ops, std::string& err);

__device__ __forceinline__ int xcd_tile(int b, int nb) {
    const int nb8 = nb & ~7;
    return b < nb8 ? (b & 7) * (nb8 >> 3) + (b >> 3) : b;
}

struct StftTables {
    const float* window;
    const float4* tw256;
    const float4* tw512;
    const double* hann64;
    const double* cs64;
    const double2* cs2;
};

constexpr int kGuardCand = 62;
constexpr int kRecIds = 4, kRecExtra = kRecIds + 2 * kGuardCand, kRecVals = kRecExtra + 4;
constexpr int kGuardRec = kRecVals + 2 * kGuardCand;
constexpr int kGuardBudget = 48;
constexpr int kGuardMaxBudget = 1024;
struct StftGuard {
    float* eps;
    int* rec;
    float* mn_lo;
    int* count;
    int cap;
    int* dirty;
    int* work;
    int* n_work;
    int* hard;
    int* n_hard;
    int hard_cap;
    const float* audio;
    int T, hop;
    StftTables tabs;
    float k_l2, k_peak;
    int* audit;
    float audit_scale;
    float slack_scale;
    int min_interval;
    int flag_cap;
};

void launch_minmax_init(float* minmax, int B, hipStream_t s);
void launch_stft512(const StftTables& tb, const float* audio, int B, int T, int hop, int W, float* spec,
                    float* minmax, hipStream_t s, bool tile_major = false, const StftGuard* guard = nullptr);
void launch_stft512_f64(const StftTables& tb, const float* audio, int B, int T, int hop, int W, float* spec, float* minmax, hipStream_t s,
                        bool tile_major = false);
void launch_spec_bytes(const float* spec, const float* minmax, int B, int W, bool tile_major, float qscale, int qzp, int8_t* out, hipStream_t s);
void launch_stft_minmax_exact(const StftTables& tb, const float* audio, int B, int T, int hop, int W, float* spec, bool tile_major,
                              const StftGuard& g, float* minmax, hipStream_t s);
void launch_stft_fix(const StftTables& tb, const float* audio, int B, int T, int hop, int W, float* spec, bool tile_major, const StftGuard& g,
                     const float* minmax, float qscale, int qzp, hipStream_t s);
bool launch_stft512_mel(const StftTables& tb, const float* audio, int B, int T, int hop, int W, float* mel_out, int M,
// ... 394 lines not shown
```

### birdnet-stm32_amd/csrc/bn_model.h

```cpp
#pragma once
#include <hip/hip_runtime.h>

#include <memory>
#include <mutex>
#include <utility>
#include <vector>

#include "../../include/birdnet_hip.h"
#include "bn_kernels.h"
#include "bn_ops.h"

namespace bn {

int fail(int code, const char* fmt, ...);
int check_device(bn_ctx* ctx);
int grow_device_buffer(void** p, size_t* have, size_t need, size_t alloc, hipStream_t s, int code, const char* what);

constexpr int kMaxGridBatch = 32768;

struct OpPrep {
    uint8_t rq_right = 0;
    bool ok = false;
    bool alt_ok = false;
    Tail8Args tail{};
    Tail2Args chain{};
    Tail2Args resident{};
};

struct SpecStage {
    bool tiled = false;
    bool guard = false;
    const float* audio = nullptr;
    int T = 0, hop = 0;
};

}

#define HIP_TRY(expr)                                                                             \
    do {                                                                                          \
        hipError_t e_ = (expr);                                                                   \
        if (e_ != hipSuccess)                                                                     \
            return bn::fail(BN_ERR_DEVICE, "%s failed: %s (%s:%d)", #expr, hipGetErrorString(e_), __FILE__, __LINE__); \
    } while (0)

struct bn_ctx {
    std::vector<std::pair<int bn::Options::*, int>> opt_override;
    int device = 0;
    int max_batch = 0;
    float* d_window = nullptr;
    float4* d_tw256 = nullptr;
    float4* d_tw512 = nullptr;
    double* d_f64tab = nullptr;
    bn::StftTables tables{};
    float* d_block_peaks = nullptr;
    size_t block_peaks_elems = 0;
    void* d_rank_work = nullptr;
    size_t rank_work_bytes = 0;
    void* d_search_work = nullptr;
    size_t search_work_bytes = 0;
    void* d_kmeans_work = nullptr;
    size_t kmeans_work_bytes = 0;
    void* d_tsne_work = nullptr;
    size_t tsne_work_bytes = 0;
    void* d_boot_work = nullptr;
    size_t boot_work_bytes = 0;
};

struct bn_model {
    bn_ctx* ctx = nullptr;
    BlobHeader hdr{};
    std::vector<OpRec> ops;
    std::vector<TensorRec> tensors;
    std::vector<SlotRec> slots;
    char* d_consts = nullptr;
    size_t consts_base = 0;
    size_t consts_bytes = 0;
    std::vector<std::unique_ptr<bn::OpPrep>> prep;
    bool has_mid = false;
    std::vector<uint8_t> out_valid;
    std::vector<uint8_t> slot_valid;
    bool has_tail = false;
    bool guard_form_ok = false;
    bool spec_tiled_ok = false;
    std::vector<char*> d_slots;
    float* d_spec = nullptr;
    float* d_minmax = nullptr;
    char* d_guard = nullptr;
    bn::StftGuard guard{};
    bool last_tiled = false;
    int last_B = 0;
    int* d_audit = nullptr;
    float* d_smax = nullptr;
    float* d_gap_part = nullptr;
    size_t gap_part_elems = 0;
    int32_t* d_pool8 = nullptr;
    size_t pool8_C = 0;
    size_t workspace_bytes = 0;
    int emb_dim = 0;
    float emb_scale = 1.0f;
    int emb_zp = 0;
    bool profiling = false;
    int prof_only = -1;
    struct EvRec {
        int op;
        hipEvent_t start, stop;
    };
    std::vector<EvRec> ev_used;
    std::vector<hipEvent_t> ev_free;

// ... 57 lines not shown
```

### birdnet-stm32_amd/csrc/bn_plan_run.hip

```cpp
#include <algorithm>
#include <cstring>

#include "bn_model.h"
#include "bn_quant_in.h"

namespace bn {

namespace {

inline bool same_path(const OpRec& head, const OpRec& partner) {
    return partner.p[BN_OP_PATH] == BN_PATH_BOTH || partner.p[BN_OP_PATH] == head.p[BN_OP_PATH];
}
inline bool on_path(const OpRec& o, int mode) { return o.p[BN_OP_PATH] == BN_PATH_BOTH || o.p[BN_OP_PATH] == mode; }
inline int tag(const OpRec& o) { return o.p[BN_OP_TAIL_TAG]; }

bool gate_pools_dw(const OpRec& d, const OpRec& g) {
    namespace k = op::f32_dw;
    namespace q = op::f32_segate;
    return g.kind == BN_OP_F32_SEGATE && g.in0 == d.out && g.p[q::C] == d.p[k::C] && g.p[q::P] == d.p[k::OH] * d.p[k::OW];
}
int pwdw_row_blocks(const OpRec& d) {
    const int OH = d.p[op::f32_dw::OH], rb = f32_pwdw_rows(OH);
    return (OH + rb - 1) / rb;
}
// ... 46 lines not shown
        const float sc = i8 ? o.f[BN_OP_EMB_SCALE] : 1.0f;
        const int zp = i8 ? p[BN_OP_EMB_ZP] : 0;
        const bool same = m->emb_dim == 0 || (m->emb_dim == width && m->emb_scale == sc && m->emb_zp == zp);
        if (width <= 0 || width % 4 || width != p[BN_OP_EMB_DIM] || i8 != (m->hdr.dtype == BN_DTYPE_I8) || !same || (i8 && !(sc > 0.0f)) ||
            zp < -128 || zp > 127 || (o.kind != BN_OP_I8_TAIL && o.kind != BN_OP_F32_GAPDENSE && o.out < 0))
            return fail(BN_ERR_FORMAT, "operator %zu (kind %d): malformed embedding mark", oi, o.kind);
        m->emb_dim = width;
        m->emb_scale = sc;
        m->emb_zp = zp;
    }
    for (const OpRec& o : m->ops)
        if (o.in0 == BN_SLOT_INPUT) {
            namespace k = op::i8_dwpw;
            m->spec_tiled_ok = o.kind == BN_OP_I8_DWPW && o.p[k::q_at_load] && o.p[k::transposed] && o.p[k::W] % 64 == 0;
            m->guard_form_ok = m->spec_tiled_ok && o.p[k::qzp] == -128;
        }
    auto all_right = [&](int t_mult, int t_shift) {
        if (t_mult < 0 || t_shift < 0) return false;
        const TensorRec& tm = m->tensors[t_mult];
        const TensorRec& ts = m->tensors[t_shift];
        const int32_t* pm = (const int32_t*)(base + tm.offset);
        const int32_t* ps = (const int32_t*)(base + ts.offset);
        if ((tm.nbytes | ts.nbytes) & 3) return false;
        for (size_t i = 0; i < tm.nbytes / 4; ++i)
            if (pm[i] < 0) return false;
        for (size_t i = 0; i < ts.nbytes / 4; ++i)
            if (ps[i] >= 0) return false;
        return true;
    };
    auto all_narrow = [&](int t_shift) {
        if (t_shift < 0) return false;
        const TensorRec& ts = m->tensors[t_shift];
        const int32_t* ps = (const int32_t*)(base + ts.offset);
        bool narrow = true;
        for (size_t i = 0; i < ts.nbytes / 4; ++i) narrow = narrow && ps[i] >= -20;
        return narrow;
    };
    m->prep.clear();
    m->prep.resize(n);
    for (size_t oi = 0; oi < n; ++oi) {
        const OpRec& o = m->ops[oi];
        const int* p = o.p;
        if (o.kind != BN_OP_I8_DWPW && o.kind != BN_OP_I8_DW && o.kind != BN_OP_I8_STEM && o.kind != BN_OP_I8_FRONT && o.kind != BN_OP_I8_TAIL &&
            o.kind != BN_OP_I8_MID)
            continue;
        m->prep[oi].reset(new OpPrep());
        OpPrep& pr = *m->prep[oi];
        if (o.kind == BN_OP_I8_DWPW) {
            namespace k = op::i8_dwpw;
            const bool pw_ok = all_right(o.t[k::pw_mult], o.t[k::pw_shift]);
            bool ok = pw_ok && (!p[k::has_dw] || all_right(o.t[k::dw_mult], o.t[k::dw_shift]));
            if (p[k::has_add])
                ok = ok && p[k::add_m1] >= 0 && p[k::add_s1] < 0 && p[k::add_m2] >= 0 && p[k::add_s2] < 0 && p[k::add_mo] >= 0 && p[k::add_so] < 0;
            const bool narrow = pw_ok && all_narrow(o.t[k::pw_shift]);
            pr.rq_right = (ok ? 1 : 0) | (narrow ? 2 : 0) | (pw_ok ? 4 : 0);
        } else if (o.kind == BN_OP_I8_DW || o.kind == BN_OP_I8_STEM) {
            namespace k = op::i8_dw;
            pr.rq_right = (all_right(o.t[k::mult], o.t[k::shift]) ? 1 : 0) | (all_narrow(o.t[k::shift]) ? 2 : 0);
        } else if (o.kind == BN_OP_I8_FRONT) {
            namespace k = op::i8_front;
            pr.rq_right = all_right(o.t[k::stem_mult], o.t[k::stem_shift]) && all_right(o.t[k::dw_mult], o.t[k::dw_shift]) &&
                          all_right(o.t[k::pw_mult], o.t[k::pw_shift]);
        } else if (o.kind == BN_OP_I8_MID) {
            namespace k = op::i8_mid;
            Tail2Args& ma = pr.chain;
            const int nl = p[k::n_layers];
            pr.ok = chain_prep(m, base, o, k::cst, k::desc, ma, [](const int32_t* d, int nw, int l, Tail2Args& a) { return tail2_plan(d, nw, l, a, true); },
                               [](const Tail2Args& a) { return tail2_const_words(a, true); }) &&
                    ma.L[nl - 1].OH * ma.L[nl - 1].OW == p[k::P_last] && ma.L[nl - 1].Cout == p[k::C_last];
            pr.resident = ma;
            pr.alt_ok = pr.ok && tail2_plan_resident(pr.resident);
            m->has_mid = m->has_mid || pr.ok;
        } else {
            namespace k = op::i8_tail;
            pr.tail.NC = pr.chain.NC = p[k::n_classes];
            pr.tail.s_fc = pr.chain.s_fc = o.f[k::s_fc];
            pr.tail.s_head = pr.chain.s_head = o.f[k::s_head];
            pr.ok = chain_prep(m, base, o, k::cst, k::desc, pr.tail, [](const int32_t* d, int nw, int l, Tail8Args& a) { return tail_plan(d, nw, l, a); },
                               [](const Tail8Args& a) { return tail_const_words(a); });
            m->has_tail = m->has_tail || pr.ok;
            if (pr.ok && o.t[k::cst2] >= 0 && o.t[k::desc2] >= 0 && (size_t)o.t[k::cst2] < m->tensors.size() && (size_t)o.t[k::desc2] < m->tensors.size())
                pr.alt_ok = chain_prep(m, base, o, k::cst2, k::desc2, pr.chain, [](const int32_t* d, int nw, int l, Tail2Args& a) { return tail2_plan(d, nw, l, a); },
                                       [](const Tail2Args& a) { return tail2_const_words(a); });
        }
    }
    for (size_t i = 0; i + 1 < n; ++i) {
        const OpRec& a = m->ops[i];
        const OpRec& b = m->ops[i + 1];
        if (a.kind == BN_OP_F32_DWPW && tag(a) == BN_PWDW_HEAD && b.kind == BN_OP_F32_DW)
            m->gap_part_elems = std::max(m->gap_part_elems, (size_t)pwdw_row_blocks(b) * (size_t)b.p[op::f32_dw::C]);
        if (a.kind == BN_OP_F32_DW && b.kind == BN_OP_F32_SEGATE && b.in0 == a.out) {
            namespace k = op::f32_dw;
            int cq = 16;
            while ((a.p[k::C] / 4) % cq) cq >>= 1;
            const int ncol = 64 / cq;
            m->gap_part_elems = std::max(m->gap_part_elems, (size_t)((a.p[k::OW] + ncol - 1) / ncol) * (size_t)((a.p[k::OH] + 3) / 4) * (size_t)a.p[k::C]);
        }
        if (a.kind == BN_OP_I8_DW && b.kind == BN_OP_I8_MEAN && mean_pools_dw8(a, b)) m->pool8_C = std::max(m->pool8_C, (size_t)a.p[op::i8_dw::C]);
    }
    return BN_OK;
}

StftGuard guard_slice(const bn_model* m, size_t b0, const SpecStage& st) {
    StftGuard g = m->guard;
    const size_t W = m->hdr.spec_width;
    g.eps += b0 * W;
    g.rec += b0 * ((W + 15) / 16) * kGuardRec;
    g.count += b0;
    g.dirty += b0;
    g.mn_lo += b0;
    g.min_interval = g_opt.stft_minint;
    const size_t group = b0 / kMaxGridBatch;
    g.work += b0 * ((W + 63) / 64);
    g.n_work += group;
    g.hard += b0;
    g.n_hard += 2 * group;
    g.audio = st.audio;
    g.T = st.T;
    g.hop = st.hop;
    g.tabs = m->ctx->tables;
    g.flag_cap = g_opt.stft_flagcap;
    const int gm = g_opt.stft_guard;
    g.k_l2 = gm == 1 ? kGuardL2Proven : gm == 2 ? kGuardL2 / 1024.0f : kGuardL2;
    g.k_peak = gm == 1 ? 0.0f : gm == 2 ? kGuardPeak / 1024.0f : kGuardPeak;
    g.audit_scale = gm == 2 ? 1024.0f : 1.0f;
    g.slack_scale = gm == 2 ? 0.0f : 1.0f;
    g.audit = g_opt.stft_audit ? m->d_audit : nullptr;
    return g;
}

namespace {

struct PlanRun {
    bn_model* const m;
    const RunArgs& a;
    const int B;
    hipStream_t const s;
    const int mode;
    const size_t n;
    const bool tail_on, mid_on;

    size_t gap_for = (size_t)-1;
    int gap_R = 0, cand_R = 0;
    size_t cand_for = (size_t)-1;
    size_t pwdw_head_done = (size_t)-1;
    size_t pwdw_done = (size_t)-1;
    size_t front2_done = (size_t)-1;
    size_t segate_done[2] = {(size_t)-1, (size_t)-1};
    size_t pool8_for = (size_t)-1;
    size_t scale_done = (size_t)-1;
    int emb_written = 0;

    size_t oi = 0;
    const OpRec* o = nullptr;
    const int* p = nullptr;
    char *in0 = nullptr, *in1 = nullptr, *out = nullptr;
    const float* mm = nullptr;
    ProfScope* prof = nullptr;

    PlanRun(bn_model* m_, const RunArgs& a_)
        : m(m_), a(a_), B(a_.B), s(a_.s), mode(a_.d_audio ? BN_PATH_AUDIO : BN_PATH_INPUT), n(m_->ops.size()), tail_on(m_->has_tail && g_opt.i8_tail),
          mid_on(m_->has_mid && g_opt.i8_mid && g_opt.i8_strip) {}

    char* slot_ptr(int id) const {
        if (id == BN_SLOT_INPUT) return (char*)a.d_input;
        if (id == BN_SLOT_AUDIO) return (char*)a.d_audio;
// ... 212 lines not shown
                    pwdw_done = oi + 1;
                    fused_into(oi + 1);
                    return BN_OK;
                }
            }
        }
        if (r.transposed && p[k::q_at_load]) {
            r.qx = (const float*)in0;
            r.qminmax = mm;
            r.qscale = o->f[k::qscale];
            r.qzp = p[k::qzp];
            r.qfill = p[k::qfill];
            r.qF = p[k::qF];
            r.qtiled = (a.spec.tiled && o->in0 == BN_SLOT_INPUT) ? 1 : 0;
            r.x = nullptr;
            if (!i8_mel_mfma_supported(r)) return fail(BN_ERR_FORMAT, "operator %zu: fused QUANTIZE needs the mel-mixer kernel's geometry", oi);
            if (a.spec.guard && r.qtiled && mm) {
                r.qguard = guard_slice(m, a.slot_b0, a.spec);
                r.qmode = 1;
                launch_i8_dwpw(r, s);
                prof->end();
                ProfScope fix(m, (int)n + 2, s);
                launch_stft_fix(m->ctx->tables, a.spec.audio, B, a.spec.T, a.spec.hop, r.W, (float*)in0, true, r.qguard, mm, r.qscale, r.qzp, s);
                r.qmode = 2;
                launch_i8_dwpw(r, s);
                return BN_OK;
            }
        }
        if (p[k::strip] && o->t[k::strip_cst] >= 0 && g_opt.i8_strip && r.has_dw && !r.transposed && r.sh == r.sw &&
            i8_strip_supported(r.Cin, r.Cout, r.sh, r.OW, r.add.enabled != 0) && (!r.add.enabled || (r.res == r.x && o->t[k::add_tab] >= 0))) {
            const int off = r.add.enabled ? 128 : 0;
            Strip8Args q{r.x, r.y, t32(*o, k::strip_cst), B, r.H, r.W, r.OH, r.OW, 0, r.pt, r.pl, r.dw_zp_in, r.dw_amin, r.dw_amax, r.pw_amin + off,
                         r.pw_amax + off, r.pw_zp_out, r.add, r.add.enabled ? t8(*o, k::add_tab) : nullptr};
            launch_i8_strip(q, r.Cin, r.Cout, r.sh, s);
            return BN_OK;
        }
        if (!i8_dwpw_supported(r.Cin, r.Cout) || r.TH * r.TW * r.NB != 64 || r.OH % r.TH || r.OW % r.TW)
            return fail(BN_ERR_FORMAT, "operator %zu: unsupported fused INT8 block geometry", oi);
        launch_i8_dwpw(r, s);
        return BN_OK;
    }

    int i8_front() {
        namespace k = op::i8_front;
        I8FrontParams q{};
        q.stem_w = t8(*o, k::stem_w); q.stem_b = t32(*o, k::stem_b); q.stem_mult = t32(*o, k::stem_mult); q.stem_shift = t32(*o, k::stem_shift);
        q.dw_w = t8(*o, k::dw_w); q.dw_b = t32(*o, k::dw_b); q.dw_mult = t32(*o, k::dw_mult); q.dw_shift = t32(*o, k::dw_shift);
        q.pw_w = t8(*o, k::pw_w); q.pw_b = t32(*o, k::pw_b); q.pw_mult = t32(*o, k::pw_mult); q.pw_shift = t32(*o, k::pw_shift);
        q.H0 = p[k::H0]; q.W0 = p[k::W0]; q.C = p[k::C]; q.N = p[k::N]; q.OH = p[k::OH]; q.OW = p[k::OW];
        q.stem_zp_in = p[k::stem_zp_in]; q.stem_zp_out = p[k::stem_zp_out]; q.stem_amin = p[k::stem_amin]; q.stem_amax = p[k::stem_amax];
        q.dw_zp_out = p[k::dw_zp_out]; q.dw_amin = p[k::dw_amin]; q.dw_amax = p[k::dw_amax];
        q.pw_zp_out = p[k::pw_zp_out]; q.pw_amin = p[k::pw_amin]; q.pw_amax = p[k::pw_amax];
        q.rq_right = m->prep[oi]->rq_right;
        if (p[k::strip] && o->t[k::strip_cst] >= 0 && g_opt.i8_strip && i8_front_strip_supported(q.H0, q.W0, q.C, q.N, q.OH, q.OW)) {
            FrontStrip8Args fa{(const int8_t*)in0, (int8_t*)out, t32(*o, k::strip_cst), B, q.H0, q.W0, q.OH, q.OW, 0, q.stem_zp_in, q.stem_amin, q.stem_amax,
                               q.stem_zp_out, q.dw_amin, q.dw_amax, q.pw_amin, q.pw_amax};
            launch_i8_front_strip(fa, s);
            return BN_OK;
        }
        if (!i8_front_supported(q.H0, q.W0, q.C, q.N, q.OH, q.OW)) return fail(BN_ERR_FORMAT, "operator %zu: unsupported INT8 front-block geometry", oi);
        launch_i8_front(q, (const int8_t*)in0, (int8_t*)out, B, s);
        return BN_OK;
    }

    int i8_mid() {
        const OpPrep& pr = *m->prep[oi];
        Tail2Args ma = g_opt.i8_mid_split && pr.alt_ok ? pr.resident : pr.chain;
        ma.x = (const int8_t*)in0;
        ma.y = (int8_t*)out;
        ma.cst = t32(*o, op::i8_mid::cst);
        ma.B = B;
        if (!launch_i8_mid2(ma, s)) return fail(BN_ERR_DEVICE, "could not raise the LDS limit of the fused stage-2 kernel");
        return BN_OK;
    }

    int i8_tail() {
        namespace k = op::i8_tail;
        const OpPrep& pr = *m->prep[oi];
        const EmbOut eo{a.d_emb, a.emb_dtype == BN_EMB_F32, p[BN_OP_EMB_ZP], o->f[BN_OP_EMB_SCALE]};
        const EmbOut* emb = emb_for(*o) ? &eo : nullptr;
        emb_written += emb != nullptr;
        bool launched;
        if (g_opt.i8_tail_mfdw && pr.alt_ok) {
            Tail2Args t2 = pr.chain;
            t2.x = (const int8_t*)in0;
            t2.scores = a.d_scores;
            t2.logits = a.d_logits;
            t2.cst = t32(*o, k::cst2);
            t2.B = B;
            launched = launch_i8_tail2(t2, s, emb);
        } else {
            Tail8Args ta = pr.tail;
            ta.x = (const int8_t*)in0;
            ta.scores = a.d_scores;
            ta.logits = a.d_logits;
            ta.cst = t32(*o, k::cst);
            ta.B = B;
            launched = launch_i8_tail(ta, s, emb);
        }
        if (!launched) return fail(BN_ERR_DEVICE, "could not raise the LDS limit of the fused tail kernel");
        return BN_OK;
    }

    int i8_mean() {
        namespace k = op::i8_mean;
        namespace f = op::i8_fc;
        if (segate_fused(oi)) {
            const OpRec& f1 = m->ops[oi + 1];
            const OpRec& f2 = m->ops[oi + 2];
            launch_i8_segate((const int8_t*)in0, (int8_t*)slot_ptr(f2.out), B, p[k::P], p[k::C], p[k::zp_in], p[k::mult], p[k::shift], p[k::zp_out],
                             f1.p[f::Cout], f1.p[f::zp_out], f1.p[f::act_min], f1.p[f::act_max], t8(f1, f::w), t32(f1, f::bias), t32(f1, f::mult), t32(f1, f::shift),
                             f1.p[f::has_lut] ? t8(f1, f::lut) : nullptr, f2.p[f::zp_out], f2.p[f::act_min], f2.p[f::act_max], t8(f2, f::w), t32(f2, f::bias),
                             t32(f2, f::mult), t32(f2, f::shift), f2.p[f::has_lut] ? t8(f2, f::lut) : nullptr, s, oi == pool8_for ? m->d_pool8 : nullptr);
            segate_done[0] = oi + 1;
            segate_done[1] = oi + 2;
            fused_into(oi + 2);
            return BN_OK;
        }
        launch_i8_mean((const int8_t*)in0, (int8_t*)out, B, p[k::P], p[k::C], p[k::zp_in], p[k::mult], p[k::shift], p[k::zp_out], s);
        return BN_OK;
    }

    int i8_scale() {
        namespace k = op::i8_scale;
        if (tag(*o) == BN_SCALE_HEAD && g_opt.i8_strip && oi + 1 < n) {
            namespace dk = op::i8_dwpw;
            const OpRec& d = m->ops[oi + 1];
            if (same_path(*o, d) && d.kind == BN_OP_I8_DWPW && tag(d) == BN_SCALE_COVERED && d.in0 == o->out && d.out != o->in0 && d.out != o->in1 &&
                d.p[dk::Cin] == p[k::C] && d.p[dk::OH] * d.p[dk::OW] == p[k::P]) {
                DwPw8Args a2 = dwpw8_args(d, oi + 1);
                a2.x = (const int8_t*)in0;
                a2.gate = (const int8_t*)in1;
                a2.g_zx = p[k::zp_x]; a2.g_zg = p[k::zp_gate]; a2.g_mult = p[k::mult]; a2.g_shift = p[k::shift]; a2.g_zo = p[k::zp_out];
                a2.g_amin = p[k::act_min]; a2.g_amax = p[k::act_max];
                if (!a2.has_dw && !a2.transposed && i8_pw_wave_takes(a2)) {
                    launch_i8_dwpw(a2, s);
                    scale_done = oi + 1;
                    fused_into(oi + 1);
                    return BN_OK;
                }
            }
        }
        launch_i8_scale((const int8_t*)in0, (const int8_t*)in1, (int8_t*)out, B, p[k::P], p[k::C], p[k::zp_x], p[k::zp_gate], p[k::mult], p[k::shift],
                        p[k::zp_out], p[k::act_min], p[k::act_max], s);
        return BN_OK;
    }

    int single_launch() {
        const float* x = (const float*)in0;
        const int8_t* x8 = (const int8_t*)in0;
        float* y = (float*)out;
        int8_t* y8 = (int8_t*)out;
        switch (o->kind) {
            case BN_OP_F32_MEL: {
                namespace k = op::f32_mel;
                if (p[k::norm]) launch_u32_fill((uint32_t*)m->d_smax, 0u, B, s);
                launch_f32_mel(x, mm, y, m->d_smax, B, p[k::F], p[k::W], p[k::M], tf(*o, k::wvals), (const int*)m->tensor(o->t[k::bands]), tf(*o, k::magp),
                               p[k::mag], p[k::norm], s);
                break;
            }
            case BN_OP_F32_STFTMEL: {
                namespace k = op::f32_stftmel;
                launch_minmax_init(m->d_minmax, B, s);
                if (!launch_stft512_mel(m->ctx->tables, a.d_audio, B, a.T, a.hop, p[k::W], y, p[k::M], tf(*o, k::wvals), (const int*)m->tensor(o->t[k::bands]),
                                        m->d_minmax, s))
                    return fail(BN_ERR_UNSUPPORTED, "the fused STFT+mel kernel takes at most 128 mel bins (got %d)", p[k::M]);
                break;
// ... 161 lines not shown
```

### include/birdnet_hip.h

```cpp
#ifndef BIRDNET_HIP_H
#define BIRDNET_HIP_H

#include <stddef.h>
#include <stdint.h>

#ifdef __cplusplus
extern "C" {
#endif

#define BN_ABI_VERSION 2

#if defined(__GNUC__)
#define BN_API __attribute__((visibility("default")))
#else
#define BN_API
#endif

#define BN_OK 0
#define BN_ERR_ARG (-1)
#define BN_ERR_DEVICE (-2)
#define BN_ERR_FORMAT (-3)
#define BN_ERR_UNSUPPORTED (-4)
#define BN_ERR_NOMEM (-5)

// ... 33 lines not shown
BN_API void bn_model_free(bn_model* model);
BN_API int bn_model_get_info(const bn_model* model, bn_model_info* out);

BN_API int bn_stft_mag(bn_ctx* ctx, const float* d_audio, int B, int T, int n_fft, int hop, int W,
                int normalize, float* d_spec, float* d_minmax, void* stream);

BN_API int bn_stft_mag_exact(bn_ctx* ctx, const float* d_audio, int B, int T, int n_fft, int hop, int W,
                      int normalize, float* d_spec, float* d_minmax, void* stream);

BN_API int bn_forward(bn_model* model, const float* d_input, const float* d_minmax, int B,
               float* d_scores, float* d_logits, void* stream);

BN_API int bn_infer_audio(bn_model* model, const float* d_audio, int B, int T, int hop,
                   float* d_scores, float* d_logits, void* stream);

#define BN_EMB_F32 0
#define BN_EMB_I8 1

BN_API int bn_model_get_embedding_info(const bn_model* model, int* dim, int* dtype, float* scale, int* zero_point);

BN_API int bn_forward_embed(bn_model* model, const float* d_input, const float* d_minmax, int B, float* d_scores,
               float* d_logits, void* d_emb, int emb_dtype, void* stream);
BN_API int bn_infer_audio_embed(bn_model* model, const float* d_audio, int B, int T, int hop, float* d_scores,
               float* d_logits, void* d_emb, int emb_dtype, void* stream);


#define BN_PCM_S16 0
#define BN_PCM_S24 1
#define BN_PCM_S32 2
#define BN_PCM_F32 3

BN_API int bn_ingest_resample(bn_ctx* ctx, const void* d_pcm, int sample_format, int channels,
                       const int64_t* d_in_off, const int64_t* d_out_off, int n_windows, int64_t max_in_len,
                       int64_t max_out_len, const float* d_taps, int up, int down, int taps_per_phase,
                       int n_pre_remove, float* d_mono, float* d_peak, void* stream);

BN_API int bn_ingest_resample_span(bn_ctx* ctx, const void* d_pcm, int sample_format, int channels, int64_t s0, int64_t n_staged,
                       int64_t n_in, int64_t o0, int64_t o1, const float* d_taps, int up, int down, int taps_per_phase,
                       int n_pre_remove, float* d_mono_window, float* d_peak, void* stream);

BN_API int bn_ingest_chunks(bn_ctx* ctx, const float* d_mono, const float* d_peak, const int64_t* d_chunk_src,
                     const int32_t* d_chunk_valid, const int32_t* d_chunk_window, int n_chunks, int chunk_len,
                     float* d_chunks, void* stream);

BN_API int bn_short_time_energy(bn_ctx* ctx, const float* d_mono, const float* d_peak, const int64_t* d_win_off, const int32_t* d_win_index,
                         const int64_t* d_frame_off, int n_windows, int frame_len, int hop, float* d_ste, void* stream);

BN_API int bn_activity_counts(bn_ctx* ctx, const float* d_x, int B, int64_t n, const int32_t* d_idx, int m, float k, int32_t* d_active,
                       float* d_stats, void* stream);

BN_API int bn_rank_orders(bn_ctx* ctx, const float* d_scores, int n_rows, int n_classes, int32_t* d_cols, int32_t* d_flat, void* stream);

BN_API int bn_chunk_peak_normalize(bn_ctx* ctx, const float* d_x, int B, int T, float eps, float* d_y, void* stream);

#define BN_POOL_AVG 0
#define BN_POOL_MAX 1
#define BN_POOL_LME 2

BN_API int bn_pool_scores(bn_ctx* ctx, const float* d_scores, const int64_t* d_file_off, int n_files, int n_classes,
                   int method, float beta, float* d_pooled, void* stream);


#define BN_SPEC_MEL 0
#define BN_SPEC_LOGMEL 1
#define BN_SPEC_MFCC 2
#define BN_MAG_NONE 0
#define BN_MAG_PWL 1
#define BN_MAG_PCEN 2
#define BN_MAG_DB 3

BN_API int bn_mel_spectrogram(bn_ctx* ctx, const float* d_audio, int B, int T, int n_fft, int hop, int W,
                       const float* d_mel_w, const int32_t* d_mel_bands, int n_mels, int mode, int mag_scale,
                       double pcen_b, const float* d_dct, int n_mfcc, float* d_work, float* d_out, void* stream);

BN_API int bn_debug_op_output(bn_model* model, int op_index, int B, void* d_dst, size_t dst_bytes,
                       size_t* bytes_per_chunk, void* stream);

BN_API int bn_debug_input_bytes(bn_model* model, int B, int8_t* d_out, void* stream);
BN_API int bn_debug_guard_stats(bn_model* model, int B, int64_t* out);
BN_API int bn_debug_tail_form(const bn_model* model, int* form, int* lds_bytes);
BN_API int bn_debug_mid_form(const bn_model* model, int* form, int* lds_bytes);
BN_API int bn_debug_mid_plan(const bn_model* model, int* out, int n);
BN_API int bn_debug_mid_split_giveups(bn_ctx* ctx, int64_t* count);

BN_API int bn_debug_requant(bn_ctx* ctx, const int32_t* d_x, const int32_t* d_mult, const int32_t* d_shift, int n, int mode,
                     int zero_point, int32_t* d_out, void* stream);

BN_API int bn_profile_enable(bn_model* model, int enable);
BN_API int bn_profile_only(bn_model* model, int op_index);
BN_API int bn_profile_collect(bn_model* model, double* total_ms, int64_t* launches, int n);

BN_API int bn_set_option(const char* name, int value);
BN_API int bn_get_option(const char* name, int* value);
BN_API int bn_ctx_set_option(bn_ctx* ctx, const char* name, int value);
BN_API int bn_ctx_get_option(bn_ctx* ctx, const char* name, int* value);
BN_API int bn_ctx_reset_options(bn_ctx* ctx);

BN_API void* bn_host_alloc_pinned(bn_ctx* ctx, size_t bytes);
BN_API int bn_host_free_pinned(void* p);

#define BN_PROBE_MAX_D 2048
#define BN_PROBE_MAX_C 4096
#define BN_PROBE_ACT_SIGMOID 0
#define BN_PROBE_ACT_SOFTMAX 1
#define BN_PROBE_OPT_ADAM 0
#define BN_PROBE_OPT_ADAMW 1
#define BN_PROBE_OPT_SGD 2
#define BN_PROBE_WORKSPACE_BYTES (256u << 20)

typedef struct bn_probe bn_probe;

BN_API int bn_head_forward(bn_ctx* ctx, const float* d_emb, int64_t n, int D, const float* d_W, const float* d_b, int C, int activation,
                    float* d_scores, void* stream);

#define BN_HEAD_I8_STEP_ROWS 64
#define BN_HEAD_I8_MIN_WG_STEPS 8
#define BN_HEAD_I8_MAX_WGS 1024
#define BN_HEAD_I8_LDS_BYTES (160 * 1024)
BN_API int bn_head_i8_forward(bn_ctx* ctx, const int8_t* d_rows, int64_t n, int D, const int8_t* d_w, const int32_t* d_bias,
                       const int32_t* d_mult, const int32_t* d_shift, int C, int zp_out, const int8_t* d_lut, int activation, float s_fc,
                       int8_t* d_logit_bytes, float* d_scores, void* stream);

BN_API int bn_head_i8_pass_classes(int D, int C);

BN_API int bn_probe_create(bn_ctx* ctx, int D, int C, int activation, int optimizer, float lr, float weight_decay, float clipnorm,
                    float dropout, uint32_t seed, int64_t total_steps, const float* d_W, const float* d_b, bn_probe** out, void* stream);
BN_API void bn_probe_destroy(bn_probe* probe);
BN_API int bn_probe_epoch(bn_probe* probe, const float* d_X, const float* d_Y, const int32_t* d_perm, int64_t n, int batch,
                   float* d_step_loss, void* stream);
BN_API int bn_probe_loss(bn_probe* probe, const float* d_X, const float* d_Y, int64_t n, float* d_out, void* stream);
BN_API int bn_probe_get(bn_probe* probe, float* d_W, float* d_b, void* stream);
BN_API int bn_probe_set(bn_probe* probe, const float* d_W, const float* d_b, void* stream);
#define BN_PROBE_LOSS_CE 0
#define BN_PROBE_LOSS_FOCAL 1
BN_API int bn_probe_set_loss(bn_probe* probe, int loss, float focal_gamma);
BN_API int bn_probe_epoch_weighted(bn_probe* probe, const float* d_X, const float* d_Y, const float* d_row_weight, const int32_t* d_perm,
                            int64_t n, int batch, float* d_step_loss, void* stream);
#define BN_PROBE_QAT_OFF 0
#define BN_PROBE_QAT_PER_CLASS 1
#define BN_PROBE_QAT_PER_TENSOR 2
BN_API int bn_probe_set_qat(bn_probe* probe, int weight_mode, int quantize_logits, float s_out, int z_out);
BN_API int bn_probe_get_quantized(bn_probe* probe, float* d_Wq, void* stream);
BN_API int bn_probe_scores(bn_probe* probe, const float* d_X, int64_t n, float* d_scores, int8_t* d_codes, void* stream);

#define BN_PROBE_SWEEP_MAX_TRIALS 64
#define BN_PROBE_SWEEP_BYTES (2048ull << 20)
#define BN_PROBE_SWEEP_CURRENT 0
#define BN_PROBE_SWEEP_SNAPSHOT 1

typedef struct bn_probe_trial {
    int32_t optimizer;
    float lr;
    float weight_decay;
    float clipnorm;
    float dropout;
    float label_smoothing;
} bn_probe_trial;

typedef struct bn_probe_sweep bn_probe_sweep;

BN_API int bn_probe_sweep_create(bn_ctx* ctx, int D, int C, int activation, int T, const bn_probe_trial* trials, uint32_t seed,
                          int64_t total_steps, const float* d_W, const float* d_b, bn_probe_sweep** out, void* stream);
BN_API void bn_probe_sweep_destroy(bn_probe_sweep* sweep);
BN_API int bn_probe_sweep_epoch(bn_probe_sweep* sweep, const float* d_X, const float* d_Y, const int32_t* d_perm, int64_t n, int batch,
                         const float* d_step_sizes, const uint8_t* d_active, float* d_step_loss, void* stream);
BN_API int bn_probe_sweep_loss(bn_probe_sweep* sweep, const float* d_X, const float* d_Y, int64_t n, const uint8_t* d_active, float* d_out,
// ... 78 lines not shown
```

Measured before the change: 2.367 million.

## Add split-resident fused tail kernel with compacted depthwise weights

Adds a split plan for the fused int8 tail chain. The early stride-1 stage layers keep their depthwise and pointwise weights resident in LDS across chunk groups, while the later stage reuses the freed map space. Depthwise A-fragments are compacted from 16-byte diagonal vectors to one byte each, and a device copy is built at model load and expanded in registers, which cuts global and LDS traffic for weight staging. Stage-3 weights are re-requested during the head so they overlap with the next group. This adds LDS-layout complexity and a per-model compact buffer, and the plan falls back to the old path when layer shapes do not fit.

```diff
diff --git a/birdnet-stm32_amd/birdnet_stm32/_hip.py b/birdnet-stm32_amd/birdnet_stm32/_hip.py
--- a/birdnet-stm32_amd/birdnet_stm32/_hip.py
+++ b/birdnet-stm32_amd/birdnet_stm32/_hip.py
@@ -15,7 +15,7 @@
     "bn_model_free", "bn_model_get_info", "bn_stft_mag", "bn_forward", "bn_infer_audio", "bn_debug_op_output",
     "bn_kernel_names", "bn_profile_enable", "bn_profile_collect", "bn_ingest_resample", "bn_ingest_chunks",
     "bn_pool_scores", "bn_mel_spectrogram", "bn_profile_only", "bn_chunk_peak_normalize", "bn_set_option", "bn_get_option", "bn_ctx_set_option", "bn_ctx_get_option", "bn_ctx_reset_options", "bn_preload_kernels", "bn_host_alloc_pinned", "bn_host_free_pinned", "bn_rank_orders",
-    "bn_blob_check", "bn_debug_requant", "bn_stft_mag_exact", "bn_debug_input_bytes", "bn_debug_guard_stats", "bn_debug_tail_form", "bn_debug_mid_form", "bn_debug_mid_plan", "bn_debug_mid_split_giveups",
+    "bn_blob_check", "bn_debug_requant", "bn_stft_mag_exact", "bn_debug_input_bytes", "bn_debug_guard_stats", "bn_debug_tail_form", "bn_debug_mid_form", "bn_debug_mid_plan", "bn_debug_mid_split_giveups", "bn_debug_tail_plan",
     "bn_forward_embed", "bn_infer_audio_embed", "bn_model_get_embedding_info", "bn_ingest_resample_span",
     "bn_head_forward", "bn_probe_create", "bn_probe_destroy", "bn_probe_epoch", "bn_probe_loss", "bn_probe_get", "bn_probe_set",
     "bn_probe_sweep_create", "bn_probe_sweep_destroy", "bn_probe_sweep_epoch", "bn_probe_sweep_loss", "bn_probe_sweep_snapshot", "bn_probe_sweep_get",
@@ -74,7 +74,7 @@
 
 OPTION_NAMES = ("f32_strip", "f32_strip_th", "f32_front_staged", "f32_front2", "f32_pwdw", "f32_tile_slice", "f32_pw_ws", "i8_pwdw", "i8_pw_lds", "i8_pw_forms", "i8_add_tab", "front_tpw", "wave_dwpw", "i8_strip", "i8_strip_mfdw", "i8_strip_th", "i8_dw_pool", "i8_tail_fclds", "i8_tail", "i8_tail_mfdw", "i8_mid",
                 "i8_mel_generic", "stft_rowmajor", "stft_exact", "stft_flagcap", "stft_guard", "stft_audit", "stft_minint", "ingest_blk", "ingest_generic")
-SCHEDULING_OPTION_NAMES = ("i8_mid_split",)
+SCHEDULING_OPTION_NAMES = ("i8_mid_split", "i8_tail_split", "i8_chain_grid")
 
 
 class BnModelInfo(ctypes.Structure):
@@ -125,6 +125,7 @@
     lib.bn_debug_tail_form.argtypes = [c_void_p, POINTER(c_int), POINTER(c_int)]
     lib.bn_debug_mid_form.argtypes = [c_void_p, POINTER(c_int), POINTER(c_int)]
     lib.bn_debug_mid_plan.argtypes = [c_void_p, POINTER(c_int), c_int]
+    lib.bn_debug_tail_plan.argtypes = [c_void_p, POINTER(c_int), c_int]
     lib.bn_debug_mid_split_giveups.argtypes = [c_void_p, POINTER(c_int64)]
     lib.bn_forward.argtypes = [c_void_p, c_void_p, c_void_p, c_int, c_void_p, c_void_p, c_void_p]
     lib.bn_infer_audio.argtypes = [c_void_p, c_void_p, c_int, c_int, c_int, c_void_p, c_void_p, c_void_p]
diff --git a/birdnet-stm32_amd/birdnet_stm32/models/runners.py b/birdnet-stm32_amd/birdnet_stm32/models/runners.py
--- a/birdnet-stm32_amd/birdnet_stm32/models/runners.py
+++ b/birdnet-stm32_amd/birdnet_stm32/models/runners.py
@@ -251,6 +251,15 @@
         parts = [(out[5 + 6 * i + 2 * k], out[6 + 6 * i + 2 * k]) for i in range(out[4]) for k in range(3) if out[6 + 6 * i + 2 * k]]
         return {"lds_bytes": out[1], "map_bytes": out[2], "bar_off": out[3], "blocks": out[4], "parts": parts}
 
+    def tail_plan(self) -> dict | None:
+        out = (ctypes.c_int * 64)()
+        _hip.check(self.lib.bn_debug_tail_plan(self.model.handle, out, 64))
+        if not out[0]:
+            return None
+        parts = [[(out[9 + 6 * i + 2 * k], out[10 + 6 * i + 2 * k]) for k in range(3)] for i in range(out[7])]
+        return {"lds_bytes": out[1], "map3_bytes": out[2], "map4_bytes": out[3], "bar_off": out[4], "mean": (out[5], out[6]), "blocks": out[7],
+                "stage3_blocks": out[8], "parts": parts}
+
     def mid_split_giveups(self) -> int:
         n = ctypes.c_int64(0)
         _hip.check(self.lib.bn_debug_mid_split_giveups(self.ctx.handle, ctypes.byref(n)))
diff --git a/birdnet-stm32_amd/csrc/bn_api.hip b/birdnet-stm32_amd/csrc/bn_api.hip
--- a/birdnet-stm32_amd/csrc/bn_api.hip
+++ b/birdnet-stm32_amd/csrc/bn_api.hip
@@ -26,7 +26,7 @@
     {"f32_strip", &bn::Options::f32_strip},       {"f32_strip_th", &bn::Options::f32_strip_th},
     {"f32_front_staged", &bn::Options::f32_front_staged}, {"f32_front2", &bn::Options::f32_front2}, {"f32_pwdw", &bn::Options::f32_pwdw}, {"f32_tile_slice", &bn::Options::f32_tile_slice}, {"f32_pw_ws", &bn::Options::f32_pw_ws}, {"i8_pwdw", &bn::Options::i8_pwdw}, {"i8_pw_lds", &bn::Options::i8_pw_lds}, {"i8_pw_forms", &bn::Options::i8_pw_forms}, {"i8_add_tab", &bn::Options::i8_add_tab}, {"front_tpw", &bn::Options::front_tpw},
     {"wave_dwpw", &bn::Options::wave_dwpw},       {"i8_strip", &bn::Options::i8_strip},
-    {"i8_strip_th", &bn::Options::i8_strip_th}, {"i8_dw_pool", &bn::Options::i8_dw_pool}, {"i8_tail_fclds", &bn::Options::i8_tail_fclds},   {"i8_tail", &bn::Options::i8_tail}, {"i8_tail_mfdw", &bn::Options::i8_tail_mfdw}, {"i8_mid", &bn::Options::i8_mid}, {"i8_mid_split", &bn::Options::i8_mid_split},
+    {"i8_strip_th", &bn::Options::i8_strip_th}, {"i8_dw_pool", &bn::Options::i8_dw_pool}, {"i8_tail_fclds", &bn::Options::i8_tail_fclds},   {"i8_tail", &bn::Options::i8_tail}, {"i8_tail_mfdw", &bn::Options::i8_tail_mfdw}, {"i8_mid", &bn::Options::i8_mid}, {"i8_mid_split", &bn::Options::i8_mid_split}, {"i8_tail_split", &bn::Options::i8_tail_split}, {"i8_chain_grid", &bn::Options::i8_chain_grid},
     {"i8_mel_generic", &bn::Options::i8_mel_generic}, {"stft_rowmajor", &bn::Options::stft_rowmajor},
     {"i8_strip_mfdw", &bn::Options::i8_strip_mfdw}, {"stft_exact", &bn::Options::stft_exact}, {"stft_flagcap", &bn::Options::stft_flagcap}, {"stft_guard", &bn::Options::stft_guard}, {"stft_audit", &bn::Options::stft_audit}, {"stft_minint", &bn::Options::stft_minint},
     {"ingest_blk", &bn::Options::ingest_blk},
@@ -286,6 +286,13 @@
         if (hipMemcpy(m->d_consts, base + lo, m->consts_bytes, hipMemcpyHostToDevice) != hipSuccess)
             return cleanup_fail(fail(BN_ERR_DEVICE, "copying constants to the device failed"));
     }
+    for (auto& pr : m->prep)
+        if (pr && pr->split_ok) {
+            if (hipMalloc(&pr->d_dwa8, pr->dwa8.size()) != hipSuccess) return cleanup_fail(fail(BN_ERR_NOMEM, "hipMalloc of %zu operand bytes failed", pr->dwa8.size()));
+            if (hipMemcpy(pr->d_dwa8, pr->dwa8.data(), pr->dwa8.size(), hipMemcpyHostToDevice) != hipSuccess)
+                return cleanup_fail(fail(BN_ERR_DEVICE, "copying constants to the device failed"));
+            pr->split.dwa8 = (const uint8_t*)pr->d_dwa8;
+        }
     const size_t mb = (size_t)ctx->max_batch;
     m->d_slots.assign(h.n_slots, nullptr);
     for (uint32_t i = 0; i < h.n_slots; ++i) {
@@ -343,6 +350,8 @@
     if (!m) return;
     if (m->ctx) (void)hipSetDevice(m->ctx->device);
     (void)hipFree(m->d_consts);
+    for (auto& pr : m->prep)
+        if (pr) (void)hipFree(pr->d_dwa8);
     for (char* p : m->d_slots) (void)hipFree(p);
     (void)hipFree(m->d_spec);
     (void)hipFree(m->d_minmax);
@@ -625,6 +634,17 @@
     for (size_t oi = 0; oi < m->ops.size(); ++oi)
         if (m->ops[oi].kind == BN_OP_I8_MID && m->prep[oi]->ok && m->prep[oi]->alt_ok) {
             if (!bn::tail2_plan_dump(m->prep[oi]->resident, out, n)) return fail(BN_ERR_ARG, "n=%d is too small for the plan", n);
+            break;
+        }
+    return BN_OK;
+}
+
+int bn_debug_tail_plan(const bn_model* m, int* out, int n) {
+    if (!m || !out || n < 1) return fail(BN_ERR_ARG, "null argument");
+    out[0] = 0;
+    for (size_t oi = 0; oi < m->ops.size(); ++oi)
+        if (m->ops[oi].kind == BN_OP_I8_TAIL && m->prep[oi]->ok && m->prep[oi]->alt_ok && m->prep[oi]->split_ok) {
+            if (!bn::tail2_split_dump(m->prep[oi]->split, out, n)) return fail(BN_ERR_ARG, "n=%d is too small for the plan", n);
             break;
         }
     return BN_OK;
diff --git a/birdnet-stm32_amd/csrc/bn_chain_plan.cpp b/birdnet-stm32_amd/csrc/bn_chain_plan.cpp
--- a/birdnet-stm32_amd/csrc/bn_chain_plan.cpp
+++ b/birdnet-stm32_amd/csrc/bn_chain_plan.cpp
@@ -195,6 +195,10 @@
     }
     const Tail2Layer& last = a.L[n_layers - 1];
     a.resident = 0;
+    a.split = 0;
+    a.n3 = 0;
+    a.dwa8 = nullptr;
+    for (int i = 0; i < n_layers; ++i) a.L[i].a8_off = 0;
     a.bar_off = -1;
     a.fcw_off = -1;
     if (mid) {
@@ -256,6 +260,107 @@
     return true;
 }
 
+bool tail2_plan_split(Tail2Args& a) {
+    constexpr int CAP = kLdsCap - kStampBytes;
+    const int n = a.n_layers;
+    if (n < 2 || n > 8) return false;
+    int n3 = 1;
+    while (n3 < n && a.L[n3].S == 1) ++n3;
+    if (n3 == n) return false;
+    for (int i = n3 + 1; i < n; ++i)
+        if (a.L[i].S != 1 || a.L[i].Cin != a.L[n3 + 1].Cin || a.L[i].Cout != a.L[n3 + 1].Cout) return false;
+    auto up16 = [](int v) { return (v + 15) & ~15; };
+    int map3 = 0, map4 = 0, a8 = 0;
+    for (int i = 0; i < n; ++i) {
+        Tail2Layer& L = a.L[i];
+        if (i < n3) map3 = std::max(map3, tail2_map_bytes(L, i == 0, kTailG));
+        else map4 = std::max(map4, kTailG * L.OH * L.OW * (L.Cout + 16));
+        if (tail2_dwa8_bytes(L) / 16 > kTail2Threads || tail2_dwc_bytes(L, i == 0) / 16 > kTail2Threads) return false;
+        if (i < n3 && tail2_pw_bytes(L) / 16 > kTail2SplitPw16) return false;
+        L.a8_off = a8;
+        a8 += tail2_dwa8_bytes(L);
+    }
+    map3 = up16(std::max(map3, tail2_map_bytes(a.L[n3], false, kTailG)));
+    map4 = up16(map4);
+    if (map4 > map3) return false;
+    int pos = map3;
+    for (int i = 0; i < n3; ++i) {
+        Tail2Layer& L = a.L[i];
+        L.dw_off = pos;
+        pos += up16(tail2_dw_bytes_compact(L, i == 0));
+        L.pw_off = pos;
+        pos += up16(tail2_pw_bytes(L));
+    }
+    Tail2Layer& F = a.L[n3];
+    F.pw_off = map3;
+    pos = std::max(pos, map3 + up16(tail2_pw_bytes(F)));
+    for (int i = n3 + 1; i < n; ++i) {
+        Tail2Layer& L = a.L[i];
+        L.dw_off = map4;
+        L.pw_off = map4 + up16(tail2_dw_bytes_compact(L, false));
+        if (L.pw_off > map3) return false;
+        pos = std::max(pos, L.pw_off + up16(tail2_pw_bytes(L)));
+    }
+    for (int i = 1; i < n; ++i) {
+        a.L[i].zp_off = pos;
+        pos += up16(a.L[i].Cin + 16);
+    }
+    a.L[0].zp_off = 0;
+    F.dw_off = pos;
+    pos += up16(tail2_dw_bytes_compact(F, false));
+    a.mean_off = pos;
+    pos += up16(kTailG * a.C);
+    a.bar_off = pos;
+    pos += 16;
+    if (pos > CAP) return false;
+    a.lds_bytes = pos;
+    a.split = 1;
+    a.n3 = n3;
+    return true;
+}
+
+long tail2_compact_bytes(const Tail2Args& a) {
+    long s = 0;
+    for (int i = 0; i < a.n_layers; ++i) s += tail2_dwa8_bytes(a.L[i]);
+    return s;
+}
+
+bool tail2_compact_build(const Tail2Args& a, const int32_t* cst, long n_words, uint8_t* out) {
+    const uint8_t* bytes = reinterpret_cast<const uint8_t*>(cst);
+    for (int i = 0; i < a.n_layers; ++i) {
+        const Tail2Layer& L = a.L[i];
+        const long nct = L.Cin / 16;
+        if (L.g_cst < 0 || (long)L.g_cst + nct * 768 > n_words) return false;
+        const uint8_t* src = bytes + 4 * (long)L.g_cst;
+        uint8_t* dst = out + L.a8_off;
+        for (long f = 0; f < nct * 3; ++f)
+            for (int lane = 0; lane < 64; ++lane) {
+                const uint8_t* v = src + (f * 64 + lane) * 16;
+                const int m = lane & 15;
+                for (int k = 0; k < 16; ++k)
+                    if (k != m && v[k] != 0) return false;
+                dst[f * 64 + lane] = v[m];
+            }
+    }
+    return true;
+}
+
+bool tail2_split_dump(const Tail2Args& a, int* out, int n) {
+    if (n < 9 + 6 * a.n_layers) return false;
+    int map3 = 0, map4 = 0;
+    for (int i = 0; i < a.n_layers; ++i) {
+        const Tail2Layer& L = a.L[i];
+        if (i < a.n3) map3 = std::max(map3, tail2_map_bytes(L, i == 0, kTailG));
+        else map4 = std::max(map4, kTailG * L.OH * L.OW * (L.Cout + 16));
+        int* o = out + 9 + 6 * i;
+        o[0] = L.dw_off; o[1] = tail2_dw_bytes_compact(L, i == 0); o[2] = L.pw_off; o[3] = tail2_pw_bytes(L); o[4] = L.zp_off; o[5] = i == 0 ? 0 : L.Cin + 16;
+    }
+    if (a.n3 < a.n_layers) map3 = std::max(map3, tail2_map_bytes(a.L[a.n3], false, kTailG));
+    out[0] = a.split; out[1] = a.lds_bytes; out[2] = map3; out[3] = map4; out[4] = a.bar_off; out[5] = a.mean_off; out[6] = kTailG * a.C;
+    out[7] = a.n_layers; out[8] = a.n3;
+    return true;
+}
+
 long tail2_const_words(const Tail2Args& a, bool mid) {
     long need = 0;
     auto upto = [&](long off, long words) { need = off + words > need ? off + words : need; };
diff --git a/birdnet-stm32_amd/csrc/bn_chain_plan.h b/birdnet-stm32_amd/csrc/bn_chain_plan.h
--- a/birdnet-stm32_amd/csrc/bn_chain_plan.h
+++ b/birdnet-stm32_amd/csrc/bn_chain_plan.h
@@ -46,6 +46,7 @@
     int res_m, res_c_lo, res_c_hi, res_k;
     int g_cst;
     int x_off, y_off, dw_off, pw_off, zp_off;
+    int a8_off;
 };
 constexpr int kMidG = 2;
 struct Tail2Args {
@@ -62,6 +63,9 @@
     int fcw_off;
     int bar_off;
     int resident;
+    int split;
+    int n3;
+    const uint8_t* dwa8;
     Tail2Layer L[8];};
 constexpr int kTail2MaxDw16 = 7 * kTail2Threads;
 BN_HOST_DEVICE inline int tail2_dw_bytes(const Tail2Layer& L, bool first) { return (L.Cin / 16) * (3 * 1024 + (first ? 8 : 5) * 64); }
@@ -69,6 +73,14 @@
 bool tail2_plan(const int32_t* desc, int n_words, int n_layers, Tail2Args& a, bool mid = false);
 bool tail2_plan_resident(Tail2Args& a);
 bool tail2_plan_dump(const Tail2Args& a, int* out, int n);
+constexpr int kTail2SplitPw16 = 3 * kTail2Threads;
+BN_HOST_DEVICE inline int tail2_dwa8_bytes(const Tail2Layer& L) { return (L.Cin / 16) * 192; }
+BN_HOST_DEVICE inline int tail2_dwc_bytes(const Tail2Layer& L, bool first) { return (L.Cin / 16) * (first ? 8 : 5) * 64; }
+BN_HOST_DEVICE inline int tail2_dw_bytes_compact(const Tail2Layer& L, bool first) { return tail2_dwa8_bytes(L) + tail2_dwc_bytes(L, first); }
+bool tail2_plan_split(Tail2Args& a);
+long tail2_compact_bytes(const Tail2Args& a);
+bool tail2_compact_build(const Tail2Args& a, const int32_t* cst, long n_words, uint8_t* out);
+bool tail2_split_dump(const Tail2Args& a, int* out, int n);
 long tail2_const_words(const Tail2Args& a, bool mid = false);
 
 }
diff --git a/birdnet-stm32_amd/csrc/bn_i8_tail2.hip b/birdnet-stm32_amd/csrc/bn_i8_tail2.hip
--- a/birdnet-stm32_amd/csrc/bn_i8_tail2.hip
+++ b/birdnet-stm32_amd/csrc/bn_i8_tail2.hip
@@ -22,6 +22,19 @@
         if (idx < n16)
             __builtin_amdgcn_global_load_lds((const __attribute__((address_space(1))) void*)(src + 4 * (size_t)idx),
                                              (__attribute__((address_space(3))) void*)(dst + (i * kTail2Threads + wave * 64) * 16), 16, 0, 0);
+    }
+}
+__device__ __forceinline__ void dw_request_compact(const Tail2Args& a, const Tail2Layer& L, bool first, unsigned char* lds, int tid) {
+    const int nct = L.Cin / 16;
+    part_request<1>(reinterpret_cast<const int32_t*>(a.dwa8 + L.a8_off), lds + L.dw_off, nct * 12, tid);
+    part_request<1>(a.cst + L.g_cst + nct * 768, lds + L.dw_off + nct * 192, nct * (first ? 32 : 20), tid);
+}
+__device__ __forceinline__ void stage3_request(const Tail2Args& a, unsigned char* lds, int tid) {
+#pragma unroll 1
+    for (int li = 0; li < a.n3; ++li) {
+        const Tail2Layer& L = a.L[li];
+        dw_request_compact(a, L, li == 0, lds, tid);
+        part_request<kTail2SplitPw16 / kTail2Threads>(a.cst + L.g_cst + tail2_dw_bytes(L, li == 0) / 4, lds + L.pw_off, tail2_pw_bytes(L) / 16, tid);
     }
 }
 __device__ unsigned g_tail2_giveups = 0;
@@ -59,7 +72,7 @@
 }
 
 template <bool EMB>
-__device__ __forceinline__ void tail2_head(const Tail2Args& a_, unsigned char* lds, int chunk0, int stamp_slot = -1) {
+__device__ __forceinline__ void tail2_head(const Tail2Args& a_, unsigned char* lds, int chunk0, int stamp_slot = -1, bool restage = false) {
 #ifdef BN_TAIL_STAMPS
     long long st[8] = {0, 0, 0, 0, 0, 0, 0, 0};
     st[0] = (long long)__builtin_amdgcn_s_memrealtime();
@@ -79,6 +92,7 @@
     const v4i af0 = gw[0], af1 = KS > 1 ? gw[64] : af0, af2 = KS > 2 ? gw[128] : af0, af3 = KS > 3 ? gw[192] : af0;
     const v4i* fc = reinterpret_cast<const v4i*>(a.cst + a.g_fcb) + (fc_wave ? wave : nct - 1) * 12 + g;
     const v4i fc_b = fc[0], fc_mu = fc[4], fc_sh = fc[8];
+    if (restage) stage3_request(a, lds, tid);
     for (int i = tid; i < kTailG * (C / 4); i += kTail2Threads) {
         const int gq = i / (C / 4), cq = i - gq * (C / 4);
         const int* src = reinterpret_cast<const int*>(lds + L.y_off + gq * a.P * pitch + 4 * cq);
@@ -151,7 +165,7 @@
 #endif
 }
 
-template <int G, int CIN, int COUT, int S, int H, int W, bool ADD, bool SRCG, bool RES = false>
+template <int G, int CIN, int COUT, int S, int H, int W, bool ADD, bool SRCG, bool RES = false, bool CPT = false>
 __device__ __forceinline__ void tail2_block(const Tail2Layer& L, const Tail2Args& a, unsigned char* lds, int chunk0, int nxi, unsigned& seq, int stamp_slot = -1) {
 #ifdef BN_TAIL_STAMPS
     long long st[8] = {0, 0, 0, 0, 0, 0, 0, 0};
@@ -174,7 +188,8 @@
     constexpr int NR = (UPW - 1) * TR * S + 3;
     constexpr int PT = S == 1 ? 1 : 0, PL = PT;
     constexpr int DWK = SRCG ? 8 : 5;
-    constexpr int W_BYTES = KS * 64 * COUT, DWA_BYTES = NCT * 3 * 1024, DWC_BYTES = NCT * DWK * 64, PWC_BYTES = NT * 5 * 64;
+    constexpr int W_BYTES = KS * 64 * COUT, DWA_BLOB = NCT * 3 * 1024, DWC_BYTES = NCT * DWK * 64, PWC_BYTES = NT * 5 * 64;
+    constexpr int DWA_BYTES = CPT ? NCT * 192 : DWA_BLOB;
     constexpr int PW16 = (W_BYTES + PWC_BYTES) / 16, PWP = (PW16 + kTail2Threads - 1) / kTail2Threads;
     int tid = threadIdx.x;
     asm volatile("" : "+v"(tid));
@@ -182,11 +197,14 @@
     const int wave = __builtin_amdgcn_readfirstlane(tid >> 6);
     const int n = lane & 15, g = lane >> 4;
 
-    if constexpr (!RES) part_request<PWP>(a.cst + L.g_cst + (DWA_BYTES + DWC_BYTES) / 4, lds + L.pw_off, PW16, tid);
+    if constexpr (!RES) part_request<PWP>(a.cst + L.g_cst + (DWA_BLOB + DWC_BYTES) / 4, lds + L.pw_off, PW16, tid);
 
     const v4i* wl = reinterpret_cast<const v4i*>(lds + L.pw_off) + lane;
     const v4i* dwa = reinterpret_cast<const v4i*>(lds + L.dw_off) + lane;
     const v4i* dwc = reinterpret_cast<const v4i*>(lds + L.dw_off + DWA_BYTES) + g;
+    const unsigned char* dwa8 = lds + L.dw_off + lane;
+    const int a8_sh = 8 * (n & 3);
+    const int a8_m0 = (n >> 2) == 0 ? -1 : 0, a8_m1 = (n >> 2) == 1 ? -1 : 0, a8_m2 = (n >> 2) == 2 ? -1 : 0, a8_m3 = (n >> 2) == 3 ? -1 : 0;
     const v4i* pwc = reinterpret_cast<const v4i*>(lds + L.pw_off + W_BYTES) + g;
     const int dw_lo = L.dw_lo, dw_hi = L.dw_hi, pw_lo = L.pw_lo, pw_hi = L.pw_hi;
 
@@ -235,7 +253,14 @@
     auto request = [&](int ct) {
         const int b = ct & 1;
 #pragma unroll
-        for (int dy = 0; dy < 3; ++dy) af[b][dy] = dwa[(ct * 3 + dy) * 64];
+        for (int dy = 0; dy < 3; ++dy) {
+            if constexpr (CPT) {
+                const int w8 = (int)dwa8[(ct * 3 + dy) * 64] << a8_sh;
+                af[b][dy] = (v4i){w8 & a8_m0, w8 & a8_m1, w8 & a8_m2, w8 & a8_m3};
+            } else {
+                af[b][dy] = dwa[(ct * 3 + dy) * 64];
+            }
+        }
 #pragma unroll
         for (int r = 0; r < NR; ++r) {
             if constexpr (SRCG) {
@@ -294,7 +319,9 @@
     }
     BN_T2STAMP(4);
     const Tail2Layer& N = a.L[nxi < 0 ? 0 : nxi];
-    if constexpr (!RES) {
+    if constexpr (!RES && CPT) {
+        if (nxi > 0) dw_request_compact(a, N, false, lds, tid);
+    } else if constexpr (!RES) {
         const int nx_n16 = nxi < 0 ? 0 : tail2_dw_bytes(N, nxi == 0) / 16;
         part_request<kTail2MaxDw16 / kTail2Threads>(a.cst + N.g_cst, lds + N.dw_off, nx_n16, tid);
     }
@@ -372,7 +399,7 @@
         (void)N;
         if (nxi > 0) chunk_barrier<WPC>(lds, a.bar_off, gch, seq);
     } else {
-        if (nxi > 0 && tid < (N.Cin + 16) / 4) reinterpret_cast<int*>(lds + N.zp_off)[tid] = (N.zp_in & 0xff) * 0x01010101;
+        if (!CPT && nxi > 0 && tid < (N.Cin + 16) / 4) reinterpret_cast<int*>(lds + N.zp_off)[tid] = (N.zp_in & 0xff) * 0x01010101;
 #ifdef BN_TAIL_STAMPS
         if (a.bar_off >= 0) chunk_barrier<WPC>(lds, a.bar_off, gch, seq);
         BN_T2STAMP(5);
@@ -433,8 +460,59 @@
     }
 }
 
-__global__ __launch_bounds__(kTail2Threads) void i8_tail2_kernel(Tail2Args a) { tail2_main<false>(a); }
-__global__ __launch_bounds__(kTail2Threads) void i8_tail2_emb_kernel(WithEmb<Tail2Args> w) { tail2_main<true>(w.a); }
+template <bool EMB>
+__device__ __forceinline__ void tail2_split_main(const Tail2Args& a) {
+    extern __shared__ __attribute__((aligned(16))) unsigned char lds[];
+    const int ngroups = (a.B + kTailG - 1) / kTailG;
+    unsigned seq = 0;
+    if (threadIdx.x < 4) reinterpret_cast<unsigned*>(lds + a.bar_off)[threadIdx.x] = 0;
+    for (int li = 1; li < a.n_layers; ++li) {
+        const Tail2Layer& L = a.L[li];
+        if ((int)threadIdx.x < (L.Cin + 16) / 4) reinterpret_cast<int*>(lds + L.zp_off)[threadIdx.x] = (L.zp_in & 0xff) * 0x01010101;
+    }
+    dw_request_compact(a, a.L[a.n3], false, lds, (int)threadIdx.x);
+    stage3_request(a, lds, (int)threadIdx.x);
+    __syncthreads();
+    for (int grp = blockIdx.x; grp < ngroups; grp += gridDim.x) {
+        const int chunk0 = grp * kTailG;
+        const bool more = grp + (int)gridDim.x < ngroups;
+#ifdef BN_TAIL_STAMPS
+        const int gi = (grp - (int)blockIdx.x) / (int)gridDim.x;
+        const bool stamped = (int)blockIdx.x < 8 && gi < 4 && g_tail2_stamps;
+#endif
+        for (int li = 0; li < a.n_layers; ++li) {
+            const Tail2Layer& L = a.L[li];
+            const int nx = li + 1 < a.n_layers && li + 1 != a.n3 ? li + 1 : -1;
+            int slot = -1;
+#ifdef BN_TAIL_STAMPS
+            if (stamped && li < 6) slot = ((int)blockIdx.x * 4 + gi) * 8 + li;
+#endif
+            if (li == a.n3) __syncthreads();
+            if (li == 0) tail2_block<kTailG, 64, 128, 2, 16, 32, false, true, true, true>(L, a, lds, chunk0, nx, seq, slot);
+            else if (li < a.n3) tail2_block<kTailG, 128, 128, 1, 8, 16, true, false, true, true>(L, a, lds, chunk0, nx, seq, slot);
+            else if (li == a.n3) tail2_block<kTailG, 128, 256, 2, 8, 16, false, false, false, true>(L, a, lds, chunk0, nx, seq, slot);
+            else tail2_block<kTailG, 256, 256, 1, 4, 8, true, false, false, true>(L, a, lds, chunk0, nx, seq, slot);
+        }
+        int hslot = -1;
+#ifdef BN_TAIL_STAMPS
+        if (stamped) hslot = ((int)blockIdx.x * 4 + gi) * 8 + 6;
+#endif
+        tail2_head<EMB>(a, lds, chunk0, hslot, more);
+        __syncthreads();
+#ifdef BN_TAIL_STAMPS
+        if (hslot >= 0 && (threadIdx.x & 63) == 0) g_tail2_stamps[((size_t)hslot * kTail2Waves + (threadIdx.x >> 6)) * 8 + 6] = (long long)__builtin_amdgcn_s_memrealtime();
+#endif
+    }
+}
+
+__global__ __launch_bounds__(kTail2Threads) void i8_tail2_kernel(Tail2Args a) {
+    if (a.split) tail2_split_main<false>(a);
+    else tail2_main<false>(a);
+}
+__global__ __launch_bounds__(kTail2Threads) void i8_tail2_emb_kernel(WithEmb<Tail2Args> w) {
+    if (w.a.split) tail2_split_main<true>(w.a);
+    else tail2_main<true>(w.a);
+}
 
 template <bool RES>
 __device__ __forceinline__ void mid2_main(const Tail2Args& a) {
@@ -519,11 +597,16 @@
     return (long)n;
 }
 
+static int chain_grid(int ngroups) {
+    const int cap = g_opt.i8_chain_grid > 0 && g_opt.i8_chain_grid < 256 ? g_opt.i8_chain_grid : 256;
+    return ngroups < cap ? ngroups : cap;
+}
+
 bool launch_i8_tail2(Tail2Args a, hipStream_t s, const EmbOut* emb) {
     const void* k = emb ? reinterpret_cast<const void*>(i8_tail2_emb_kernel) : reinterpret_cast<const void*>(i8_tail2_kernel);
     if (!ensure_dynamic_lds(k, 160 * 1024)) return false;
     const int ngroups = (a.B + kTailG - 1) / kTailG;
-    const int grid = ngroups < 256 ? ngroups : 256;
+    const int grid = chain_grid(ngroups);
     if (emb)
         hipLaunchKernelGGL(i8_tail2_emb_kernel, dim3(grid), dim3(kTail2Threads), (size_t)a.lds_bytes, s, WithEmb<Tail2Args>{a, *emb});
     else
@@ -534,7 +617,7 @@
 bool launch_i8_mid2(Tail2Args a, hipStream_t s) {
     if (!ensure_dynamic_lds(reinterpret_cast<const void*>(i8_mid2_kernel), 160 * 1024)) return false;
     const int ngroups = (a.B + kMidG - 1) / kMidG;
-    const int grid = ngroups < 256 ? ngroups : 256;
+    const int grid = chain_grid(ngroups);
     hipLaunchKernelGGL(i8_mid2_kernel, dim3(grid), dim3(kTail2Threads), (size_t)a.lds_bytes, s, a);
     return true;
 }
diff --git a/birdnet-stm32_amd/csrc/bn_kernels.h b/birdnet-stm32_amd/csrc/bn_kernels.h
--- a/birdnet-stm32_amd/csrc/bn_kernels.h
+++ b/birdnet-stm32_amd/csrc/bn_kernels.h
@@ -37,6 +37,8 @@
     int i8_mel_generic = 0;
     int stft_rowmajor = 0;
     int i8_mid_split = 1;
+    int i8_tail_split = 1;
+    int i8_chain_grid = 0;
     int i8_strip_mfdw = 1;
     int stft_exact = 2;
     int stft_guard = 0;
diff --git a/birdnet-stm32_amd/csrc/bn_model.h b/birdnet-stm32_amd/csrc/bn_model.h
--- a/birdnet-stm32_amd/csrc/bn_model.h
+++ b/birdnet-stm32_amd/csrc/bn_model.h
@@ -25,6 +25,10 @@
     Tail8Args tail{};
     Tail2Args chain{};
     Tail2Args resident{};
+    bool split_ok = false;
+    Tail2Args split{};
+    std::vector<uint8_t> dwa8;
+    void* d_dwa8 = nullptr;
 };
 
 struct SpecStage {
diff --git a/birdnet-stm32_amd/csrc/bn_plan_run.hip b/birdnet-stm32_amd/csrc/bn_plan_run.hip
--- a/birdnet-stm32_amd/csrc/bn_plan_run.hip
+++ b/birdnet-stm32_amd/csrc/bn_plan_run.hip
@@ -152,6 +152,15 @@
             if (pr.ok && o.t[k::cst2] >= 0 && o.t[k::desc2] >= 0 && (size_t)o.t[k::cst2] < m->tensors.size() && (size_t)o.t[k::desc2] < m->tensors.size())
                 pr.alt_ok = chain_prep(m, base, o, k::cst2, k::desc2, pr.chain, [](const int32_t* d, int nw, int l, Tail2Args& a) { return tail2_plan(d, nw, l, a); },
                                        [](const Tail2Args& a) { return tail2_const_words(a); });
+            if (pr.alt_ok) {
+                pr.split = pr.chain;
+                const TensorRec& tc = m->tensors[o.t[k::cst2]];
+                pr.split_ok = tail2_plan_split(pr.split);
+                if (pr.split_ok) {
+                    pr.dwa8.assign((size_t)tail2_compact_bytes(pr.split), 0);
+                    pr.split_ok = tail2_compact_build(pr.split, (const int32_t*)(base + tc.offset), (long)(tc.nbytes / 4), pr.dwa8.data());
+                }
+            }
         }
     }
     for (size_t i = 0; i + 1 < n; ++i) {
@@ -530,7 +539,7 @@
         emb_written += emb != nullptr;
         bool launched;
         if (g_opt.i8_tail_mfdw && pr.alt_ok) {
-            Tail2Args t2 = pr.chain;
+            Tail2Args t2 = g_opt.i8_tail_split && pr.split_ok ? pr.split : pr.chain;
             t2.x = (const int8_t*)in0;
             t2.scores = a.d_scores;
             t2.logits = a.d_logits;
diff --git a/include/birdnet_hip.h b/include/birdnet_hip.h
--- a/include/birdnet_hip.h
+++ b/include/birdnet_hip.h
@@ -139,6 +139,7 @@
 BN_API int bn_debug_mid_form(const bn_model* model, int* form, int* lds_bytes);
 BN_API int bn_debug_mid_plan(const bn_model* model, int* out, int n);
 BN_API int bn_debug_mid_split_giveups(bn_ctx* ctx, int64_t* count);
+BN_API int bn_debug_tail_plan(const bn_model* model, int* out, int n);
 
 BN_API int bn_debug_requant(bn_ctx* ctx, const int32_t* d_x, const int32_t* d_mult, const int32_t* d_shift, int n, int mode,
                      int zero_point, int32_t* d_out, void* stream);
```

After: 2.391 million, median of 6. No clear change (+1.0%).
